# Rikorose/DeepFilterNet

Hardware: AMD Instinct MI355X
Metric: 48 kHz audio frames/sec (hop=480), DeepFilterNet3 enhance() (higher is better)
Workload: dtype f32 (storage and accumulation; GRU projections / recurrences, the fused DF-encoder convolutions and the pointwise halves of the ERB separable convolutions as fp16-split MFMAs: x = hi + lo in f16, hi*hi + hi*lo + lo*hi on v_mfma_f32_16x16x32_f16, ~2^-21 relative; see exact_fp32_ms_per_step); 1 GPU; DeepFilterNet3 (recalled shipped shape, conv_ch=64) enhance(pad=True), batch=256 clips x 10 s @48 kHz per GPU, 1002 STFT frames per clip; batch_per_gpu=256, global_batch=256, parallelism=clips sharded over 1 GPU(s); no collective, inputs_resident_in_hbm=True

## Files before the change

deepfilternet_amd/csrc/dfx_model.hip:

```cpp
#include "dfx_manifest.h"
#include "dfx_nn_kernels.h"

#include <cmath>
#include <functional>
#include <atomic>
#include <map>
#include <mutex>
#include <type_traits>
#include <fcntl.h>
#include <sys/file.h>
#include <sys/stat.h>
#include <unistd.h>

static int check_cfg(const dfx_model_cfg *c) {
    if (!c) DFX_FAIL(DFX_ERR_INVALID_ARG, "null model cfg");
    if (c->conv_ch != 16 && c->conv_ch != 32 && c->conv_ch != 64)
        DFX_FAIL(DFX_ERR_UNSUPPORTED, "conv_ch=%d: the HIP kernels are instantiated for 16, 32, 64", c->conv_ch);
    if (c->emb_hidden_dim != 256 || c->df_hidden_dim != 256) DFX_FAIL(DFX_ERR_UNSUPPORTED, "GRU hidden size must be 256");
    if (c->nb_erb <= 0 || c->nb_erb % 8 || c->nb_erb > 64) DFX_FAIL(DFX_ERR_UNSUPPORTED, "nb_erb must be a multiple of 8, <= 64");
    static_assert(2 * DFX_DEC10_SMEM(64, 64) <= 160 * 1024, "conv_ch <= 64, nb_erb <= 64: dfx_k_erb_dec10 must fit every accepted shape");
    if (c->nb_df <= 0 || c->nb_df % 2 || c->nb_df > c->fft_size / 2 + 1) DFX_FAIL(DFX_ERR_UNSUPPORTED, "nb_df must be even and <= F");
    if (c->df_order <= 0 || c->df_order > 16 || c->df_lookahead < 0 || c->df_lookahead >= c->df_order)
        DFX_FAIL(DFX_ERR_UNSUPPORTED, "need 0 <= df_lookahead < df_order <= 16");
    if (c->conv_lookahead < 0) DFX_FAIL(DFX_ERR_INVALID_ARG, "conv_lookahead < 0");
// ... 296 lines not shown
        if ((f & G.mask[e]) != G.want[e]) continue;
        const float *sp = G.src[e] + b * G.row[e];
        float *dp = G.dst[e] + b * G.row[e];
        for (int64_t i = threadIdx.x; i < G.row[e]; i += blockDim.x) dp[i] = sp[i];
    }
}

__global__ void dfx_k_gate_c0_shift(const unsigned char *flags, float *c0_win, int64_t B, int64_t T, int kt, int64_t frame) {
    const int64_t b = blockIdx.x;
    if (b >= B || !(flags[b] & DFX_GATE_DF)) return;
    float *w = c0_win + (b * T + T - kt) * frame;
    for (int64_t i = (int64_t)blockIdx.y * blockDim.x + threadIdx.x; i < frame; i += (int64_t)gridDim.y * blockDim.x)
        for (int j = 0; j + 1 < kt; ++j) w[j * frame + i] = w[(j + 1) * frame + i];
}

__global__ void dfx_k_gate_hold(const unsigned char *flags, float *win, int64_t cap, int64_t row, int64_t pos, int64_t h, int64_t B) {
    const int64_t b = blockIdx.x;
    if (b >= B || !(flags[b] & DFX_GATE_FROZEN)) return;
    float *w = win + (b * cap + pos) * row;
    for (int64_t i = (int64_t)blockIdx.y * blockDim.x + threadIdx.x; i < row; i += (int64_t)gridDim.y * blockDim.x)
        for (int64_t j = h - 1; j >= 0; --j) w[(j + 1) * row + i] = w[j * row + i];
}

__global__ void dfx_k_gate_pend_commit(const unsigned char *flags, unsigned char *par, int *cnt, int64_t B) {
    const int64_t b = (int64_t)blockIdx.x * blockDim.x + threadIdx.x;
    if (b >= B || !(flags[b] & DFX_GATE_DF)) return;
    par[b] ^= 1;
    cnt[b] += 1;
}

__global__ void dfx_k_gate_finish(const unsigned char *flags, int *skip_counter, float *y, int64_t y_stride, int hop, float *lsnr_out,
                                  int64_t lsnr_stride, int64_t B, int warm) {
    const int64_t b = blockIdx.x;
    if (b >= B) return;
    const unsigned char f = flags[b];
    if (f & DFX_GATE_FROZEN) {
        for (int i = threadIdx.x; i < hop; i += blockDim.x) y[b * y_stride + i] = 0.f;
        if (threadIdx.x == 0 && lsnr_out) lsnr_out[b * lsnr_stride] = (f & DFX_GATE_PAUSED) ? __int_as_float(0x7fc00000) : -15.f;
    } else if (threadIdx.x == 0 && !warm) {
        skip_counter[b] = (f & (DFX_GATE_GAINS | DFX_GATE_ZEROS)) ? 0 : skip_counter[b] + 1;
    }
}

enum { EV_START = 0, EV_C0, EV_C1, EV_C0P, EV_EMB, EV_COEFS, EV_FRONT, EV_DONE, EV_XA, EV_MASK, EV_FIN, EV_TICKET };

struct DfxCan {
    bool fuse_c0 = false;
    bool c0_batch_unfused = false;
    bool c0_h3 = false;
    bool c0_presplit = false;
    bool pw_h3 = false;
    bool fan = false, fan_skp = false;
    bool enc_fan = false;
    bool dfenc = false;
    bool fuse_enc = false;
    bool erb_tail = false;
    bool erb_enc4 = false;
    int df_out = DFX_PLAN_DF_OUT_GGEMM;
};

struct DfxSyncLayout {
    static constexpr size_t LG = (size_t)DFX_MAX_GRU_LAYERS * DFX_SEQ_GMAX;
    static constexpr size_t ready = 0;
    static constexpr size_t emb = 8;
    static constexpr size_t probe = 13;
    static constexpr size_t poison = 14;
    static constexpr size_t done = 16;
    static constexpr size_t pcnt = done + LG;
    static constexpr size_t yprog = pcnt + 16;
    static constexpr size_t giprog = yprog + LG;
    static constexpr size_t xtab = giprog + LG;
    static constexpr size_t xstat = xtab + 3 * LG;
    static constexpr size_t total = xstat + 64;
};

struct dfx_model {
    dfx_model_cfg cfg{};
    float *d_w = nullptr;
    size_t n_w = 0;
    size_t erb0_w = 0, erb0_b = 0;
    PwW erb1, erb2, erb3, dfc0, dfc1, ct3, ct2, ct1;
    size_t co_w = 0, co_ska = 0, co_skb = 0;
    float co_bias = 0.f;
    size_t tail_w0h3 = 0, tail_woh3 = 0;
    float tail_w0_unscale = 1.f, tail_wo_unscale = 1.f;
    GlinW fc_emb, enc_in, enc_out, dec_in, dec_out, dfg_in, df_skip, df_out, enc_skip, dec_skip;
    std::vector<GruW> enc_gru, dec_gru, df_gru;
    size_t lsnr_w = 0;
    float lsnr_b = 0.f;
    size_t fan_w = 0;
    int fan_chunks = 0;
    size_t efan_w1 = 0, efan_w2 = 0;
    int efan_groups = 0;
    size_t dfenc_fc = 0, dfenc_in = 0;
    float dfenc_fc_unscale = 1.f, dfenc_in_unscale = 1.f;
    size_t dfo_h3 = 0;
    float dfo_unscale = 1.f;
    size_t cp_w1 = 0, cp_w2 = 0, cp_b = 0;
    size_t cp_weff = 0, cp_b16 = 0;
    size_t cin_weff = 0, cin_b = 0;
    size_t c0_h3 = 0, dfc1_h3 = 0, cp_h3 = 0;
    float c0_unscale = 1.f, dfc1_unscale = 1.f, cp_unscale = 1.f;
    int cp_G = 0, cp_NO = 0;
    DfxLane *lanes = nullptr;
    struct DfxLaneSet *laneset = nullptr;
    hipEvent_t ev_fork = nullptr;
    hipEvent_t ev_pass = nullptr;
    hipEvent_t ev_gate = nullptr;
    mutable bool pass_pending = false;
    bool enqueue_ahead = false;
    bool concurrent = false;
    int max_chunks = 1;
    int tchunks = 12;
    int tchunk_min = 32;
    bool run_df = true;
    bool exact_fp32 = false;
    DfxCan can;
    unsigned int *d_sync = nullptr;
    unsigned int *d_psync = nullptr;
    mutable unsigned int seq_pbase = 0;
    mutable int64_t passes_ps = 0;
    mutable int64_t passes_pair = 0;
    mutable int64_t last_plan = 0;
    mutable int64_t passes_seq = 0, passes_ev = 0;
    mutable unsigned int seq_base = 0;
    unsigned long long *d_trace = nullptr;
    mutable int trace_dims[3] = {0, 0, 0};
    bool gru_seq = true;
    struct {
        int chunks = 0;
        bool gru_pair_far = false;
        bool gru_pair = true;
        int convp_late = -1;
        int p0_ahead = 3;
        int tail_every = 1;
        int dftail_every = 0;
        bool tail_split = true;
        int64_t convp_elems = (int64_t)1 << 29;
        bool c0_presplit = true;
        bool seq_trace = false;
        char hwq_probe_mode = 0;
        bool erb_enc_split = false;
        int ws_fill = -1;
    } sw;
    unsigned int *d_err = nullptr;
    unsigned int *h_err = nullptr;
    bool check_every_pass = false;
    int spin_limit = DFX_SYNC_SPIN_LIMIT;
    bool hwq_probe_pending = false;
    int hwq_probe = -1;
    const float *p(size_t off) const { return d_w + off; }
};

namespace {
struct Prep {
    const float *blob;
    const DfxManifest &man;
    std::vector<float> out;
    std::string err;
    bool exact_fp32 = false;
    struct Packed {
        bool pw = false, tail = false, c0 = false, fan = false, fan_skp = false, encfan = false, dfenc = false;
        int dfo_tiles = 0;
    } packed;
    const float *get(const std::string &name, const DfxTensor **tt = nullptr) {
        const DfxTensor *t = man.find(name);
        if (!t) {
            err = "tensor not in manifest: " + name;
            return nullptr;
        }
        if (tt) *tt = t;
        return blob + t->offset;
    }
    size_t alloc(size_t n) {
        size_t off = (out.size() + 3) & ~(size_t)3;
        out.resize(off + n, 0.f);
        return off;
    }
    bool bn(const std::string &p, int n, std::vector<float> &scale, std::vector<float> &shift) {
        const float *g = get(p + ".weight"), *b = get(p + ".bias"), *m = get(p + ".running_mean"), *v = get(p + ".running_var");
        if (!g || !b || !m || !v) return false;
        scale.resize(n);
        shift.resize(n);
        for (int i = 0; i < n; ++i) {
            const float s = g[i] / sqrtf(v[i] + 1e-5f);
            scale[i] = s;
            shift[i] = b[i] - m[i] * s;
        }
        return true;
    }
};

bool prep_sep(Prep &P, const std::string &name, int C, PwW &w) {
    const float *dw = P.get(name + ".0.weight"), *pw = P.get(name + ".1.weight");
    std::vector<float> sc, sh;
    if (!dw || !pw || !P.bn(name + ".2", C, sc, sh)) return false;
    w.dw = P.alloc(3 * C);
    w.wt = P.alloc((size_t)C * C);
    w.bias = P.alloc(C);
    for (int c = 0; c < C; ++c)
        for (int j = 0; j < 3; ++j) P.out[w.dw + j * C + c] = dw[c * 3 + j];
    for (int n = 0; n < C; ++n)
        for (int k = 0; k < C; ++k) P.out[w.wt + (size_t)k * C + n] = pw[(size_t)n * C + k] * sc[n];
    for (int n = 0; n < C; ++n) P.out[w.bias + n] = sh[n];
    return true;
}
// ... 286 lines not shown
    }
    const DfxLane &ln = m->lanes[0];
    std::vector<hipStream_t> ss;
    if (ln.gs[1]) ss.push_back(ln.gs[1]);
    for (int i = 0; i < DFX_MAX_GRU_LAYERS; ++i)
        if (ln.ps[i]) ss.push_back(ln.ps[i]);
    for (int i = 0; i < 2; ++i)
        if (ln.ts[i]) ss.push_back(ln.ts[i]);
    unsigned int *cnt = m->d_sync + DfxSyncLayout::probe;
    for (hipStream_t st : ss) dfx_launch(dfx_k_probe_meet, dim3(1), dim3(64), 0, st, cnt, 0u, 1, m->d_err + 9);
    bool okp = hipGetLastError() == hipSuccess;
    for (hipStream_t st : ss) okp = hipStreamSynchronize(st) == hipSuccess && okp;
    m->hwq_probe = 0;
    for (int attempt = 0; attempt < 2 && okp && m->hwq_probe == 0; ++attempt) {
        (void)hipMemset(cnt, 0, sizeof(unsigned int));
        m->h_err[8] = 0u;
        for (hipStream_t st : ss) dfx_launch(dfx_k_probe_meet, dim3(1), dim3(64), 0, st, cnt, (unsigned int)ss.size(), 1 << (16 + 3 * attempt), m->d_err + 8);
        okp = hipGetLastError() == hipSuccess;
        for (hipStream_t st : ss) okp = hipStreamSynchronize(st) == hipSuccess && okp;
        m->hwq_probe = okp && ((volatile unsigned int *)m->h_err)[8] == 0u ? 1 : 0;
    }
    m->h_err[8] = 0u, m->h_err[9] = 0u;
    (void)hipMemset(cnt, 0, sizeof(unsigned int));
    if (ls) ls->hwq_probe = m->hwq_probe;
    if (m->hwq_probe == 0) hwq_probe_fallback(m);
}

namespace {
bool prep_erb_conv0(Prep &P, dfx_model *m) {
    const int C = m->cfg.conv_ch;
    const float *w = P.get("enc.erb_conv0.1.weight");
    std::vector<float> sc, sh;
    if (!w || !P.bn("enc.erb_conv0.2", C, sc, sh)) return false;
    m->erb0_w = P.alloc(9 * C);
    m->erb0_b = P.alloc(C);
    for (int ch = 0; ch < C; ++ch) {
        for (int k = 0; k < 9; ++k) P.out[m->erb0_w + k * C + ch] = w[ch * 9 + k] * sc[ch];
        P.out[m->erb0_b + ch] = sh[ch];
    }
    return true;
}
bool prep_df_conv0(Prep &P, dfx_model *m) {
    const int C = m->cfg.conv_ch;
    const float *w = P.get("enc.df_conv0.1.weight"), *pw = P.get("enc.df_conv0.2.weight");
    std::vector<float> sc, sh;
    if (!w || !pw || !P.bn("enc.df_conv0.3", C, sc, sh)) return false;
    m->cin_weff = P.alloc((size_t)20 * C);
    m->cin_b = P.alloc(C);
    for (int n = 0; n < C; ++n) {
        for (int tap = 0; tap < 9; ++tap)
            for (int ch = 0; ch < 2; ++ch) {
                double acc = 0.0;
                for (int c = ch * (C / 2); c < (ch + 1) * (C / 2); ++c) acc += (double)pw[(size_t)n * C + c] * (double)w[c * 9 + tap];
                P.out[m->cin_weff + (size_t)(tap * 2 + ch) * C + n] = (float)(acc * (double)sc[n]);
            }
        P.out[m->cin_b + n] = sh[n];
    }
    return true;
}
bool prep_lsnr(Prep &P, dfx_model *m) {
    const float *w = P.get("enc.lsnr_fc.0.weight"), *b = P.get("enc.lsnr_fc.0.bias");
    if (!w || !b) return false;
    const int emb = m->cfg.conv_ch * m->cfg.nb_erb / 4;
    m->lsnr_w = P.alloc(emb);
    memcpy(&P.out[m->lsnr_w], w, sizeof(float) * emb);
    m->lsnr_b = b[0];
    return true;
}
bool prep_conv0_out(Prep &P, dfx_model *m) {
    const int C = m->cfg.conv_ch;
    const float *w = P.get("erb_dec.conv0_out.0.weight");
    std::vector<float> sc, sh;
    if (!w || !P.bn("erb_dec.conv0_out.1", 1, sc, sh)) return false;
    m->co_w = P.alloc(3 * C);
    for (int ch = 0; ch < C; ++ch)
        for (int j = 0; j < 3; ++j) P.out[m->co_w + j * C + ch] = w[ch * 3 + j] * sc[0];
    m->co_bias = sh[0];
    return true;
}
void pack_tail_h3(Prep &P, dfx_model *m) {
    const int C = m->cfg.conv_ch;
    if (C % 32 != 0) return;
    const int KC = C / 32;
    const size_t w0 = m->erb0_w, b0 = m->erb0_b, wo = m->co_w;
    m->tail_w0h3 = pack_h3(P, C / 16, [&](int nt, int l, int i) {
        const int k = 8 * (l >> 4) + i, ch = 16 * nt + (l & 15);
        return k < 9 ? P.out[w0 + (size_t)k * C + ch] : (k == 9 ? P.out[b0 + ch] : 0.f);
    }, &m->tail_w0_unscale);
    m->tail_woh3 = pack_h3(P, KC, [&](int kc, int l, int i) {
        const int j = l & 15, e = 8 * kc + i, ch = 16 * (e >> 2) + 4 * (l >> 4) + (e & 3);
        return j < 3 ? P.out[wo + (size_t)j * C + ch] : 0.f;
    }, &m->tail_wo_unscale);
    P.packed.tail = true;
}
bool prep_df_convp(Prep &P, dfx_model *m) {
    const dfx_model_cfg &c = m->cfg;
    const int C = c.conv_ch, kt = c.df_pathway_kernel_size_t, NO = 2 * c.df_order, G = dfx_gcd(C, NO), CG = C / G, OG = NO / G;
    const int idx = kt > 1 ? 1 : 0;
    const bool has_pw = kt > 1;
    const float *w = P.get("df_dec.df_convp." + std::to_string(idx) + ".weight");
    const float *pw = has_pw ? P.get("df_dec.df_convp." + std::to_string(idx + 1) + ".weight") : nullptr;
    std::vector<float> sc, sh;
    if (!w || (has_pw && !pw) || !P.bn("df_dec.df_convp." + std::to_string(idx + (has_pw ? 2 : 1)), NO, sc, sh)) return false;
    m->cp_G = G;
    m->cp_NO = NO;
    m->cp_w1 = P.alloc((size_t)G * kt * CG * 16);
    m->cp_w2 = P.alloc((size_t)NO * NO);
    m->cp_b = P.alloc(NO);
    for (int g = 0; g < G; ++g)
        for (int k = 0; k < kt; ++k)
            for (int ci = 0; ci < CG; ++ci)
                for (int o = 0; o < OG; ++o) {
                    float v = w[(((size_t)(g * OG + o) * CG + ci) * kt + k)];
                    if (!has_pw) v *= sc[g * OG + o];
                    P.out[m->cp_w1 + ((((size_t)g * kt + k) * CG + ci) * 16 + o)] = v;
                }
    for (int n = 0; n < NO; ++n) {
        for (int o = 0; o < NO; ++o) P.out[m->cp_w2 + (size_t)n * NO + o] = has_pw ? pw[(size_t)n * NO + o] * sc[n] : (n == o ? 1.f : 0.f);
        P.out[m->cp_b + n] = sh[n];
    }
    const bool folded = NO <= 16;
    m->cp_weff = P.alloc(folded ? (size_t)kt * C * 16 : 0);
    m->cp_b16 = P.alloc(16);
    for (int k = 0; folded && k < kt; ++k)
        for (int ch = 0; ch < C; ++ch) {
            const int g = ch / CG, ci = ch - g * CG;
            for (int n = 0; n < NO; ++n) {
                double acc = 0.0;
                for (int o = g * OG; o < (g + 1) * OG; ++o) {
                    const double p2 = has_pw ? (double)pw[(size_t)n * NO + o] : (n == o ? 1.0 : 0.0);
                    acc += p2 * (double)w[((size_t)o * CG + ci) * kt + k];
                }
                P.out[m->cp_weff + ((size_t)k * C + ch) * 16 + n] = (float)(acc * (double)sc[n]);
            }
        }
    for (int n = 0; folded && n < NO; ++n) P.out[m->cp_b16 + n] = sh[n];
    return true;
}
void pack_c0_h3(Prep &P, dfx_model *m) {
    const dfx_model_cfg &c = m->cfg;
    const int C = c.conv_ch, kt = c.df_pathway_kernel_size_t;
    if (C % 32 != 0 || 2 * c.df_order > 16) return;
    const int KC = C / 32;
    auto chan = [](int kc, int l, int i) { const int e = 8 * kc + i; return 16 * (e >> 2) + 4 * (l >> 4) + (e & 3); };
    const size_t cin = m->cin_weff, wt1 = m->dfc1.wt, cpw = m->cp_weff;
    m->c0_h3 = pack_h3(P, C / 16, [&](int nt, int l, int i) {
        const int k = 8 * (l >> 4) + i;
        return k < 18 ? P.out[cin + (size_t)k * C + 16 * nt + (l & 15)] : 0.f;
    }, &m->c0_unscale);
    m->dfc1_h3 = pack_h3(P, (C / 16) * KC, [&](int fr, int l, int i) {
        const int nt = fr / KC, kc = fr % KC;
        return P.out[wt1 + (size_t)chan(kc, l, i) * C + 16 * nt + (l & 15)];
    }, &m->dfc1_unscale);
    m->cp_h3 = pack_h3(P, kt * KC, [&](int fr, int l, int i) {
        const int k = fr / KC, kc = fr % KC;
        return P.out[cpw + ((size_t)k * C + chan(kc, l, i)) * 16 + (l & 15)];
    }, &m->cp_unscale);
    P.packed.c0 = true;
}
void pack_dfo_h3(Prep &P, dfx_model *m) {
    const GlinW a = m->df_out;
    const int NO = 2 * m->cfg.df_order, Fd = m->cfg.nb_df;
    if (!(a.Kg <= 32 && a.Kg % 8 == 0 && a.Ng % 2 == 0 && NO % 2 == 0 && Fd % 2 == 0 && (int64_t)a.G * a.Ng == (int64_t)NO * Fd &&
          DFX_DFO_SMEM(NO, Fd) <= (size_t)64 * 1024))
        return;
    const int NU = (a.Ng + 15) / 16;
    m->dfo_h3 = pack_h3(P, a.G * NU, [&](int fr, int l, int i) {
        const int g = fr / NU, u = fr % NU, o = 16 * u + (l & 15), k = 8 * (l >> 4) + i;
        return o < a.Ng && k < a.Kg ? P.out[a.w + ((size_t)g * a.Kg + k) * a.Ng + o] : 0.f;
    }, &m->dfo_unscale);
    P.packed.dfo_tiles = NU;
// ... 165 lines not shown
        } else if (m->sw.hwq_probe_mode != '0') {
            m->hwq_probe_pending = true;
        }
    }
    *out = m;
    return DFX_OK;
}

static void pass_gate_forget(const dfx_model *m);
extern "C" void dfx_model_free(dfx_model *m) {
    if (!m) return;
    pass_gate_forget(m);
    if (m->ev_fork) (void)hipEventDestroy(m->ev_fork);
    if (m->ev_pass) (void)hipEventDestroy(m->ev_pass);
    if (m->ev_gate) (void)hipEventDestroy(m->ev_gate);
    dfx_env_err_words_free(m->h_err);
    if (m->d_sync && m->d_trace) {
        unsigned int n = 0;
        if (hipMemcpy(&n, m->d_sync + DfxSyncLayout::xstat, sizeof(n), hipMemcpyDeviceToHost) == hipSuccess) fprintf(stderr, "[dfx] same-XCD (light) block hand-overs over the model's life: %u\n", n);
    }
    if (m->d_sync) (void)hipFree(m->d_sync);
    if (m->d_psync) (void)hipFree(m->d_psync);
    if (m->d_trace) (void)hipFree(m->d_trace);
    if (m->d_w) (void)hipFree(m->d_w);
    delete m;
}
extern "C" int dfx_model_set_streams(dfx_model *m, int enable) {
    if (!m) DFX_FAIL(DFX_ERR_INVALID_ARG, "null");
    m->concurrent = enable != 0;
    return DFX_OK;
}
extern "C" int dfx_model_set_run_df(dfx_model *m, int enable) {
    if (!m) DFX_FAIL(DFX_ERR_INVALID_ARG, "null");
    m->run_df = enable != 0;
    return DFX_OK;
}
extern "C" int dfx_model_set_pipeline(dfx_model *m, int time_chunks, int min_chunk_frames, int batch_chunks) {
    if (!m || time_chunks < 1 || min_chunk_frames < 1 || batch_chunks < 1) DFX_FAIL(DFX_ERR_INVALID_ARG, "dfx_model_set_pipeline: bad arguments");
    m->tchunks = time_chunks < DFX_MAX_TCHUNKS ? time_chunks : DFX_MAX_TCHUNKS;
    m->tchunk_min = min_chunk_frames;
    m->max_chunks = batch_chunks < DFX_MAX_LANES ? batch_chunks : DFX_MAX_LANES;
    for (int l = 1; l < m->max_chunks; ++l)
        if (!dfx_create_lane(m, l)) DFX_FAIL(DFX_ERR_HIP, "dfx_model_set_pipeline: could not create the streams of lane %d", l);
    return DFX_OK;
}
static int model_poll(const dfx_model *m) {
    unsigned int *h = m->h_err;
    if (!h) return DFX_OK;
    if (!(((volatile unsigned int *)h)[1] | ((volatile unsigned int *)h)[2])) return DFX_OK;
    const unsigned int e1 = __atomic_exchange_n(&h[1], 0u, __ATOMIC_ACQ_REL), e2 = __atomic_exchange_n(&h[2], 0u, __ATOMIC_ACQ_REL);
    if (!(e1 | e2)) return DFX_OK;
    if (e2)
        DFX_FAIL(DFX_ERR_HIP, "dfx: a flag wait of the persistent GRU phase timed out (bounded spin: the streams of the pass did not make progress "
                              "independently — hardware queues shared with other work, or the GPU shared with another process); the results of "
                              "the previous pass on this model are invalid.  DFX_GRU_SEQ=0 selects the event-synchronised form");
    DFX_FAIL(DFX_ERR_UNSUPPORTED, "dfx: an activation of magnitude >= 6e4 reached an fp16-split matrix kernel (GRU / DF-encoder / separable-conv "
                                  "path); the results of the previous pass on this model are invalid.  DFX_EXACT_FP32=1 selects the exact fp32 kernels");
}
extern "C" int dfx_model_poll(const dfx_model *m) {
    if (!m) DFX_FAIL(DFX_ERR_INVALID_ARG, "null");
    return model_poll(m);
}
extern "C" int dfx_model_check(const dfx_model *m) {
    if (!m) DFX_FAIL(DFX_ERR_INVALID_ARG, "null");
    DFX_HIP(hipDeviceSynchronize());
    return model_poll(m);
}
extern "C" int dfx_model_query(const dfx_model *m, int what, int64_t *value) {
    if (!m || !value) DFX_FAIL(DFX_ERR_INVALID_ARG, "dfx_model_query: null");
    switch (what) {
        case DFX_Q_GRU_PERSISTENT:
        case DFX_Q_HWQ_PROBE: {
            std::lock_guard<std::mutex> lk(dfx_enqueue_mu());
            hwq_probe_run(const_cast<dfx_model *>(m));
            *value = what == DFX_Q_HWQ_PROBE ? m->hwq_probe : (m->gru_seq && m->concurrent ? 1 : 0);
            return DFX_OK;
        }
        case DFX_Q_EXACT_FP32: *value = m->exact_fp32 ? 1 : 0; return DFX_OK;
        case DFX_Q_PASSES_PERSISTENT: *value = m->passes_seq; return DFX_OK;
        case DFX_Q_PASSES_TICKET_BUSY: *value = m->passes_ev; return DFX_OK;
        case DFX_Q_SPIN_LIMIT: *value = m->spin_limit; return DFX_OK;
        case DFX_Q_PASSES_C0_PRESPLIT: *value = m->passes_ps; return DFX_OK;
        case DFX_Q_LAST_PLAN: *value = m->last_plan; return DFX_OK;
        case DFX_Q_PASSES_PAIR: *value = m->passes_pair; return DFX_OK;
    }
    DFX_FAIL(DFX_ERR_INVALID_ARG, "dfx_model_query: unknown item %d", what);
}
extern "C" int dfx_model_seq_trace(const dfx_model *m, unsigned long long *out_host, int64_t cap, int *dims) {
    if (!m || !m->d_trace || !out_host || !dims) DFX_FAIL(DFX_ERR_INVALID_ARG, "dfx_model_seq_trace: tracing is off (DFX_SEQ_TRACE=1 at model creation)");
    const int64_t n = (int64_t)m->trace_dims[0] * m->trace_dims[1] * m->trace_dims[2] * 3;
    if (n > cap) DFX_FAIL(DFX_ERR_INVALID_ARG, "dfx_model_seq_trace: buffer too small");
    DFX_HIP(hipMemcpy(out_host, m->d_trace, (size_t)n * 8, hipMemcpyDeviceToHost));
    for (int i = 0; i < 3; ++i) dims[i] = m->trace_dims[i];
    return DFX_OK;
}
extern "C" int dfx_model_cfg_get(const dfx_model *m, dfx_model_cfg *out) {
    if (!m || !out) DFX_FAIL(DFX_ERR_INVALID_ARG, "null");
    *out = m->cfg;
    return DFX_OK;
}

static inline bool dfx_dfenc_ok(const dfx_model *m, int64_t B, int64_t T, int64_t feat_T) {
    const dfx_model_cfg &c = m->cfg;
    const int64_t emb = (int64_t)c.conv_ch * c.nb_erb / 4;
    return m->can.dfenc && B * T * emb < ((int64_t)1 << 31) && B * (feat_T > 0 ? feat_T : T) * c.nb_df < ((int64_t)1 << 29);
}
static inline bool dfx_feat_spec_unread(const dfx_model *m, int64_t B, int64_t T) { return m->can.c0_presplit && dfx_dfenc_ok(m, B, T, 0); }
static inline float *dfx_ws_base(void *workspace) { return reinterpret_cast<float *>(((uintptr_t)workspace + 255) & ~(uintptr_t)255); }

namespace {
struct Ws {
    size_t e0, e1, e2, e3, c0, c1, emb_in, emb, xa, xb, gi, xa2, xb2, gi2, demb, d3, d2, mask, c0p, xdf, coefs, lsnr, skp_e, skp_d, fps, total;
    size_t pgi[DFX_MAX_GRU_LAYERS], py[DFX_MAX_GRU_LAYERS], ph[DFX_MAX_GRU_LAYERS];
};
Ws plan_ws(const dfx_model *m, int64_t R, int64_t B) {
    const dfx_model_cfg &c = m->cfg;
    const bool c0_stored = !m->can.fuse_c0 || m->can.c0_batch_unfused, presplit = m->can.c0_presplit;
    Ws w{};
    size_t off = 0;
    auto take = [&](size_t n) {
        size_t o = off;
        off += (n + 63) & ~(size_t)63;
        return o;
    };
    const size_t C = c.conv_ch, E = c.nb_erb, Fd = c.nb_df, emb = C * E / 4, NO = 2 * c.df_order;
    w.e0 = take(R * E * C);
    w.e1 = take(R * (E / 2) * C);
    w.e2 = take(R * (E / 4) * C);
    w.e3 = take(R * (E / 4) * C);
    w.c0 = c0_stored ? take(R * Fd * C) : 0;
    w.c1 = take(R * (Fd / 2) * C);
    w.emb_in = take(R * emb * (c.enc_concat ? 2 : 1));
    w.emb = take(R * emb);
    w.xa = take(R * 256);
    w.xb = take(R * 256);
    w.gi = take(R * 768);
    w.xa2 = take(R * 256);
    w.xb2 = take(R * 256);
    w.gi2 = take(R * 768);
    w.demb = take(R * emb);
    w.d3 = take(R * (E / 4) * C);
    w.d2 = take(R * (E / 2) * C);
    w.mask = take(R * E);
    w.c0p = take(R * Fd * NO);
    w.xdf = take(R * 256);
    w.coefs = take(R * Fd * NO);
    w.lsnr = take(R);
    w.skp_e = take(c.emb_gru_skip_enc == DFX_SKIP_GROUPEDLINEAR ? R * emb : 0);
    w.skp_d = take(c.emb_gru_skip == DFX_SKIP_GROUPEDLINEAR ? R * emb : 0);
    w.fps = take(presplit ? R * Fd * 2 : 0);
    const int nlayers = 1 + (c.emb_num_layers - 1) + c.df_num_layers;
    for (int l = 0; l < DFX_MAX_GRU_LAYERS; ++l) {
        const bool used = l < nlayers;
        w.pgi[l] = take(used ? R * 768 : 0);
        w.py[l] = take(used ? R * 256 : 0);
        w.ph[l] = take(used ? (B > 0 ? B : R) * 256 : 0);
    }
    w.total = off;
    return w;
}
}

extern "C" int dfx_model_workspace_bytes(const dfx_model *m, int64_t B, int64_t T, int64_t *bytes) {
    if (!m || !bytes || B < 0 || T < 0) DFX_FAIL(DFX_ERR_INVALID_ARG, "dfx_model_workspace_bytes: bad arguments");
    *bytes = (int64_t)(plan_ws(m, B * T, B).total * sizeof(float)) + 256;
    return DFX_OK;
}

#include "dfx_model_launch.h"
#include "dfx_model_forward.h"
#include "dfx_model_stream.h"
#include "dfx_stream_move.h"
#include "dfx_model_enhance.h"
```

deepfilternet_amd/csrc/dfx_model_forward.h:

```cpp
#pragma once

#ifdef DFX_DEV
static int dfx_dev_skip() {
    static const int v = [] { const char *e = getenv("DFX_DEV_SKIP"); return e ? atoi(e) : 0; }();
    return v;
}
static bool dfx_dev_stage(int n) {
    static const int lo = [] { const char *e = getenv("DFX_DEV_STAGE_LO"); return e ? atoi(e) : 0; }();
    static const int hi = [] { const char *e = getenv("DFX_DEV_STAGE_HI"); return e ? atoi(e) : 99; }();
    return n >= lo && n <= hi;
}
#else
static constexpr int dfx_dev_skip() { return 0; }
static constexpr bool dfx_dev_stage(int) { return true; }
#endif

struct TicketGuard {
    bool armed = false;
    ~TicketGuard() {
        if (armed) dfx_ticket_release_cb(nullptr);
    }
};

template <int C>
struct DfxPass {
    const dfx_model *m;
    const dfx_bands *bands;
    const float *spec, *feat_erb, *feat_spec;
    int64_t B, T;
    float atten_lim;
    float *spec_e, *ws;
    hipStream_t s;
    const DfxLane *ln;
    bool signal_front;
    const DfxFinish *fin;
    const DfxStreamCtx *sc;
    const dfx_model_cfg &c;
    int64_t R, t_begin, Rn, featT, t_zero, sstride;
    DfxRowMap rmw;
    int Lk, E, Fd, O, NO, emb, L, kt;
    const int *tzr;
    Ws w{};
    float *e0, *e1, *e2, *e3, *c0, *c1, *emb_in, *embv, *xa, *xb, *gi, *demb, *d3, *d2, *mask, *c0p, *xdf, *coefs, *lsnr, *xa2, *xb2, *gi2, *skp_e, *skp_d;
    bool run_df, fan, fan_skp, par, c0_fused, fuse_h3, fuse_tail, fuse_enc, no_e0, fuse_enc4, enc_fan, dfenc, pipe, use_seq;
    hipStream_t x1, x2;
    hipStream_t fin_s;
    const float *cp_feat, *e0r;
    const uint2 *fps;
    const DfxGate *gate;
    int nenc, ndec, ndf, nl, groups;
    int K = 0;
    int cb[DFX_GS_MAX_CHUNKS + 1];
    int64_t convp_split;
    TicketGuard ticket_guard;

    int plan(float *mask_out, float *lsnr_out, float *coefs_out) {
        R = B * T;
        if (R >= ((int64_t)1 << 31)) DFX_FAIL(DFX_ERR_UNSUPPORTED, "forward: %lld x %lld frames in one call (32-bit row index)", (long long)B, (long long)T);
        t_begin = sc ? sc->H : 0, Rn = B * (T - t_begin);
        featT = sc ? sc->feat_T : 0;
        rmw = sc ? DfxRowMap{T, T - t_begin, t_begin} : DfxRowMap{0, 0, 0};
        Lk = sc ? 0 : c.conv_lookahead;
        t_zero = sc ? sc->t_zero : 0;
        tzr = sc ? sc->t_zero_rows : nullptr;
        w = plan_ws(m, R, B);
        sstride = fin ? fin->spec_stride : 0;
        fin_s = s;
        E = c.nb_erb, Fd = c.nb_df, O = c.df_order, NO = 2 * O, emb = C * E / 4, L = c.conv_lookahead;
        e0 = ws + w.e0, e1 = ws + w.e1, e2 = ws + w.e2, e3 = ws + w.e3, c0 = ws + w.c0, c1 = ws + w.c1;
        emb_in = ws + w.emb_in, embv = ws + w.emb, xa = ws + w.xa, xb = ws + w.xb, gi = ws + w.gi;
        demb = ws + w.demb, d3 = ws + w.d3, d2 = ws + w.d2;
        mask = mask_out ? mask_out : ws + w.mask;
        c0p = ws + w.c0p, xdf = ws + w.xdf;
        coefs = coefs_out ? coefs_out : ws + w.coefs;
        lsnr = lsnr_out ? lsnr_out : ws + w.lsnr;
        xa2 = ws + w.xa2, xb2 = ws + w.xb2, gi2 = ws + w.gi2;
        skp_e = ws + w.skp_e, skp_d = ws + w.skp_d;
        run_df = m->run_df;
        fan = m->can.fan;
        fan_skp = m->can.fan_skp && run_df;
        par = m->concurrent;
        x1 = par ? ln->aux[0] : s, x2 = par ? ln->aux[1] : s;
        c0_fused = m->can.fuse_c0 && !(m->can.c0_batch_unfused && !sc);
        if (sc && !c0_fused) DFX_FAIL(DFX_ERR_UNSUPPORTED, "streaming needs the fused DF encoder (df_pathway_kernel_size_t <= 5, df_order <= 8)");
        cp_feat = c0_fused ? feat_spec : nullptr;
        fuse_h3 = c0_fused && m->can.c0_h3;
        fps = !sc && m->can.c0_presplit ? reinterpret_cast<const uint2 *>(ws + w.fps) : nullptr;
        fuse_tail = m->can.erb_tail, fuse_enc = m->can.fuse_enc;
        no_e0 = fuse_tail && fuse_enc;
        fuse_enc4 = m->can.erb_enc4 && !sc && !m->sw.erb_enc_split;
        e0r = no_e0 ? nullptr : e0;
        if (sc && !fuse_enc) DFX_FAIL(DFX_ERR_UNSUPPORTED, "streaming needs the fused ERB encoder head (nb_erb even and <= 62, a frame's rows within the LDS)");
        gate = sc ? sc->gate : nullptr;
        if (gate && T - t_begin != 1) DFX_FAIL(DFX_ERR_INVALID_ARG, "gated streaming passes carry exactly one new frame");
        kt = c.df_pathway_kernel_size_t;
        convp_split = T;
        enc_fan = m->can.enc_fan;
        dfenc = fuse_h3 && dfx_dfenc_ok(m, B, T, featT);
        K = m->tchunks;
        if (T / K < m->tchunk_min) K = (int)(T / m->tchunk_min);
        nenc = (int)m->enc_gru.size(), ndec = (int)m->dec_gru.size(), ndf = run_df ? (int)m->df_gru.size() : 0;
        pipe = par && !sc && K > 1 && nenc == 1 && 1 + ndec + ndf <= DFX_MAX_GRU_LAYERS && ln == &m->lanes[0];
        nl = 1 + ndec + ndf;
        groups = (int)dfx_ceil_div(B, DFX_GH_ROWS);
        if (pipe && m->gru_seq && m->hwq_probe_pending && groups <= DFX_SEQ_GMAX && nl * groups + 8 <= dfx_env_num_cus())
            hwq_probe_run(const_cast<dfx_model *>(m));
        const bool want_seq = pipe && m->gru_seq && groups <= DFX_SEQ_GMAX && nl * groups + 8 <= dfx_env_num_cus();
        use_seq = want_seq && dfx_ticket_try();
        m->passes_seq += use_seq ? 1 : 0, m->passes_ev += (want_seq && !use_seq) ? 1 : 0;
        ticket_guard.armed = use_seq && dfx_ticket().fd >= 0;
        if (use_seq) {
            const int kbody = m->sw.chunks > 0 ? m->sw.chunks : 12;
            const int64_t body = std::max<int64_t>(dfx_ceil_div(T, (int64_t)kbody), m->tchunk_min);
            K = (int)std::max<int64_t>(1, std::min<int64_t>(dfx_ceil_div(T, body), DFX_GS_MAX_CHUNKS));
        }
        if (pipe)
            for (int i = 0; i <= K; ++i) cb[i] = (int)(T * i / K);
        m->last_plan = (fan ? DFX_PLAN_FAN : 0) | (fan_skp ? DFX_PLAN_FAN_SKP : 0) | (fuse_h3 ? DFX_PLAN_FUSE_H3 : 0) |
                       (c0_fused && fps ? DFX_PLAN_PRESPLIT : 0) | (fuse_tail ? DFX_PLAN_FUSE_TAIL : 0) | (fuse_enc ? DFX_PLAN_FUSE_ENC : 0) |
                       (fuse_enc4 ? DFX_PLAN_FUSE_ENC4 : 0) | (enc_fan ? DFX_PLAN_ENC_FAN : 0) | (dfenc ? DFX_PLAN_DFENC : 0) |
                       (c0_fused ? DFX_PLAN_C0_FUSED : 0) | (pipe ? DFX_PLAN_PIPE : 0) | (use_seq ? DFX_PLAN_USE_SEQ : 0) |
                       DFX_PLAN_FUSE_DEC;
        return DFX_OK;
    }
    void note_df_out(int form) const { m->last_plan = (m->last_plan & ~(int64_t)DFX_PLAN_DF_OUT_MASK) | ((int64_t)form << DFX_PLAN_DF_OUT_SHIFT); }
    int64_t tb(int k) const { return cb[k]; }
    DfxRowMap rmk(int k0, int k) const { return DfxRowMap{T, tb(k + 1) - tb(k0), tb(k0)}; }
    DfxRowMap rmk(int k) const { return rmk(k, k); }
    int64_t Mk(int k0, int k) const { return B * (tb(k + 1) - tb(k0)); }
    int64_t Mk(int k) const { return Mk(k, k); }

    int signal(int e, hipStream_t from) {
        if (par) DFX_HIP(hipEventRecord(ln->ev[e], from));
        return DFX_OK;
    }
    int wait(int e, hipStream_t on) {
        if (par) DFX_HIP(hipStreamWaitEvent(on, ln->ev[e], 0));
        return DFX_OK;
    }
    int ewait(hipEvent_t e, hipStream_t on) {
        DFX_HIP(hipStreamWaitEvent(on, e, 0));
        return DFX_OK;
    }
    int esig(hipEvent_t e, hipStream_t from) {
        DFX_HIP(hipEventRecord(e, from));
        return DFX_OK;
    }
    int enc_skip_res(const float **res, int64_t M, hipStream_t st, DfxRowMap rm) {
        *res = c.emb_gru_skip_enc == DFX_SKIP_IDENTITY ? emb_in : c.emb_gru_skip_enc == DFX_SKIP_GROUPEDLINEAR ? skp_e : nullptr;
        return *res == skp_e ? launch_glin(m, m->enc_skip, emb_in, DFX_ACT_NONE, nullptr, skp_e, M, st, rm) : DFX_OK;
    }
    int enc_out_skip(const float *y, int64_t M, hipStream_t st, DfxRowMap rm) {
        const float *res;
        if (int r = enc_skip_res(&res, M, st, rm)) return r;
        return launch_glin(m, m->enc_out, y, DFX_ACT_RELU, res, embv, M, st, rm);
    }
    int dec_out_skip(const float *y, int64_t M, hipStream_t st, DfxRowMap rm) {
        const float *res = nullptr;
        if (c.emb_gru_skip == DFX_SKIP_IDENTITY) res = embv;
        else if (c.emb_gru_skip == DFX_SKIP_GROUPEDLINEAR) {
            if (int r = launch_glin(m, m->dec_skip, embv, DFX_ACT_NONE, nullptr, skp_d, M, st, rm)) return r;
            res = skp_d;
        }
        return launch_glin(m, m->dec_out, y, DFX_ACT_RELU, res, demb, M, st, rm);
    }
    int emb_fan(const float *y, float *dec_x, int64_t M, hipStream_t st, DfxRowMap rm, const DfxPublish *pub = nullptr) {
        const float *res;
        if (int r = enc_skip_res(&res, M, st, rm)) return r;
        const bool need_emb = c.emb_gru_skip != DFX_SKIP_NONE || (run_df && c.df_gru_skip == DFX_SKIP_IDENTITY);
        return launch_emb_fan(m, y, res, need_emb ? embv : nullptr, dec_x, run_df ? xa2 : nullptr, fan_skp ? xdf : nullptr, lsnr, M, st, rm, embv, pub);
    }
    int df_out_rows(const float *cfeat, const float *cfeat2, int64_t M, hipStream_t st, DfxRowMap rm) {
        if (m->can.df_out != DFX_PLAN_DF_OUT_GGEMM && M > 0 && R * (int64_t)NO * Fd < ((int64_t)1 << 31)) {
            DfxDfOutArgs A;
            A.a = cfeat, A.a2 = cfeat2;
            A.wf = reinterpret_cast<const dfx_h8 *>(m->p(m->dfo_h3));
            A.c0p = c0p, A.out = coefs;
            A.R = M, A.T = T;
            A.G = m->df_out.G, A.Kg = m->df_out.Kg, A.Ng = m->df_out.Ng, A.NO = NO, A.Fd = Fd;
            A.unscale = m->dfo_unscale;
            A.rm = rm;
            A.err = m->d_err;
            const size_t smem = DFX_DFO_SMEM(NO, Fd);
            DfxKScope ks(DFX_K_GGEMM, st);
            const bool resident = m->can.df_out == DFX_PLAN_DF_OUT_RESIDENT;
            note_df_out(m->can.df_out);
            if (resident) {
                DFX_HIP(dfx_env_set_max_dyn_smem((const void *)dfx_k_df_out_h3r<4>, smem));
                dfx_launch(dfx_k_df_out_h3r<4>, dim3((unsigned)nn_grid(dfx_ceil_div(M, 16), 2)), dim3(DFX_DFO_THREADS), smem, st, A);
            } else {
                DFX_HIP(dfx_env_set_max_dyn_smem((const void *)dfx_k_df_out_h3, smem));
                dfx_launch(dfx_k_df_out_h3, dim3((unsigned)nn_grid(dfx_ceil_div(M, 16), 2)), dim3(DFX_DFO_THREADS), smem, st, A);
            }
            DFX_LAUNCH_CHECK();
            return DFX_OK;
        }
        note_df_out(DFX_PLAN_DF_OUT_GGEMM);
        return launch_ggemm(cfeat, m->df_out.G * m->df_out.Kg, m->p(m->df_out.w), m->df_out.G, m->df_out.Kg, m->df_out.Ng, nullptr, DFX_ACT_TANH,
                            c0p, coefs, m->df_out.G * m->df_out.Ng, M, st, NO, Fd, T, rm, cfeat2);
    }
    int erb_dec_convs(int64_t M, DfxRowMap rm, hipStream_t st) {
        int r;
        if (fuse_tail) return launch_erb_tail<C>(m, demb, e3, e2, e1, e0r, mask, M, E, st, rm, feat_erb, T, featT, Lk);
        if ((r = launch_pw<C>(DFX_PW_MODE_DW3, m, m->ct3, demb, e3, d3, M, E / 4, E / 4, 1, st, rm))) return r;
        if ((r = launch_pw<C>(DFX_PW_MODE_DWT3, m, m->ct2, d3, e2, d2, M, E / 4, E / 2, 2, st, rm))) return r;
        return launch_erb_dec10<C>(m, d2, e1, e0, mask, M, E, st, rm);
    }
    int df_skip_identity(const float *y, hipStream_t st) {
        DfxKScope ks(DFX_K_ADD, st);
        dfx_launch(dfx_k_add, dim3((unsigned)nn_grid(dfx_ceil_div(R * 256, 256), 16)), dim3(256), 0, st, y, (const float *)embv, xdf, R * 256);
        DFX_LAUNCH_CHECK();
        return DFX_OK;
    }
    int df_tail_rows(const float *y, int64_t M, DfxRowMap rm, hipStream_t st, bool join_c0p = false) {
        int r;
        const float *cfeat = y, *cfeat2 = nullptr;
        if (fan_skp) {
            cfeat2 = xdf;
        } else if (c.df_gru_skip == DFX_SKIP_GROUPEDLINEAR) {
            if ((r = launch_glin(m, m->df_skip, embv, DFX_ACT_NONE, y, xdf, M, st, rm))) return r;
            cfeat = xdf;
        } else if (c.df_gru_skip == DFX_SKIP_IDENTITY) {
            if ((r = df_skip_identity(y, st))) return r;
            cfeat = xdf;
        }
        if (join_c0p && (r = wait(EV_C0P, st))) return r;
        return df_out_rows(cfeat, cfeat2, M, st, rm);
    }
    int df_tail_identity(const float *y, hipStream_t st) {
        if (int r = df_skip_identity(y, st)) return r;
        note_df_out(DFX_PLAN_DF_OUT_GGEMM);
        return launch_ggemm(xdf, m->df_out.G * m->df_out.Kg, m->p(m->df_out.w), m->df_out.G, m->df_out.Kg, m->df_out.Ng, nullptr, DFX_ACT_TANH,
                            c0p, coefs, m->df_out.G * m->df_out.Ng, R, st, NO, Fd, T);
    }
    int lsnr_all(hipStream_t st) {
        DfxKScope ks(DFX_K_LSNR, st);
        dfx_launch(dfx_k_lsnr, dim3((unsigned)dfx_ceil_div(R * 64, 256)), dim3(256), 0, st, (const float *)embv, m->p(m->lsnr_w), m->lsnr_b,
                   (float)(c.lsnr_max - c.lsnr_min), (float)c.lsnr_min, lsnr, R, emb);
        DFX_LAUNCH_CHECK();
        return DFX_OK;
    }
    int proj_chunk(const GruW &g, int l, int k, const float *xin, hipStream_t st, const DfxPublish *pub = nullptr) {
        if (m->exact_fp32) {
            const int r = launch_proj(xin, m->p(g.wih_t), m->p(g.bias_i), ws + w.pgi[l], Mk(k), 768, st, rmk(k));
            return r || !pub ? r : launch_flag_set(pub->flag, pub->value, st);
        }
        return launch_proj_h3(m, g, xin, ws + w.pgi[l], Mk(k), 768, st, rmk(k), pub);
    }
    int conv_in_df(float *out, int lookahead, int64_t t0, int64_t rows, hipStream_t st) {
        DfxCinArgs A;
        A.feat = feat_spec, A.weff = m->p(m->cin_weff), A.bias = m->p(m->cin_b), A.out = out;
        A.B = B, A.T = T, A.Fin = Fd, A.L = lookahead;
        A.t_begin = t0, A.out_T = T, A.out_toff = t0;
        DfxKScope ks(DFX_K_CONV_IN_DF, st);
        dfx_launch(dfx_k_conv_in_df<C>, dim3((unsigned)nn_grid(dfx_ceil_div(rows * Fd, 64), 8)), dim3(DFX_PW_THREADS), 0, st, A);
        DFX_LAUNCH_CHECK();
        return DFX_OK;
    }
    int df1_range(int64_t t0, int64_t t1, hipStream_t st) {
        if (fuse_h3) return launch_conv01_h3<C>(m, m->dfc1, feat_spec, c1, B, T, Fd, Fd / 2, 2, st, t0, Lk, t1, featT);
        return launch_conv01<C>(m, m->dfc1, feat_spec, c1, B, T, Fd, Fd / 2, 2, st, t0, Lk, t1);
    }
    int convp_range(int64_t t0, int64_t t1, hipStream_t st) {
        if (dfx_dev_skip() & 8) return DFX_OK;
        if (gate && kt > 1 && gate->pend2 && fuse_h3 && t1 - t0 == 1 && t1 == T)
            return dfx_with_kt<2>(kt, [&](auto k) {
                return launch_convp_step<C, decltype(k)::value>(m, feat_spec, c0p, B, T, Fd, NO, st, t_zero, Lk, gate->pend2, 0, false, featT, gate->par, gate->cnt, tzr);
            });
        if (gate && kt > 1) {
            if (kt > 5) DFX_FAIL(DFX_ERR_UNSUPPORTED, "gated streaming needs df_pathway_kernel_size_t <= 5");
            if (int r = conv_in_df(gate->c0_win, Lk, T - 1, B, st)) return r;
            return dfx_with_kt<2>(kt, [&](auto k) { return launch_convp2<C, decltype(k)::value>(m, gate->c0_win, nullptr, c0p, B, T, Fd, NO, st, T - 1, 0, Lk); });
        } else if (fuse_h3 && sc && sc->c0ring && !gate && t1 - t0 == 1 && t1 == T && kt >= 2) {
            sc->c0ring_used = true;
            return dfx_with_kt<2>(kt, [&](auto k) {
                return launch_convp_step<C, decltype(k)::value>(m, feat_spec, c0p, B, T, Fd, NO, st, t_zero, Lk, sc->c0ring, sc->c0slot, sc->c0rebuild, featT, nullptr, nullptr, tzr);
            });
        } else if (fuse_h3) {
            return dfx_with_kt<1>(kt, [&](auto k) { return launch_convp_h3<C, decltype(k)::value>(m, feat_spec, c0p, B, T, Fd, NO, st, t0, t_zero, Lk, t1, featT, tzr, fps); });
        } else if (kt <= 5 && NO <= 16) {
            return dfx_with_kt<1>(kt, [&](auto k) { return launch_convp2<C, decltype(k)::value>(m, c0, cp_feat, c0p, B, T, Fd, NO, st, t0, t_zero, Lk, t1, tzr); });
        }
        DfxCpArgs A;
        A.c0 = c0;
        A.w1 = m->p(m->cp_w1);
        A.w2 = m->p(m->cp_w2);
        A.bias = m->p(m->cp_b);
        A.out = c0p;
        A.B = B;
        A.T = T;
        A.Fd = Fd;
        A.kt = kt;
        A.G = m->cp_G;
        A.NO = NO;
        A.tchunks = (int)dfx_ceil_div(T, DFX_CP_TT);
        A.fchunks = (Fd + DFX_CP_FB - 1) / DFX_CP_FB;
        const int CG = C / A.G;
        const size_t smem = ((size_t)(DFX_CP_TT + A.kt - 1) * DFX_CP_FB * (C + 2) + (size_t)A.G * A.kt * CG * 16 +
                             (size_t)DFX_CP_TT * DFX_CP_FB * NO) * sizeof(float);
        if (smem > 64 * 1024) DFX_HIP(dfx_env_set_max_dyn_smem((const void *)dfx_k_df_convp<C>, smem));
        const int64_t nblk = B * A.tchunks * A.fchunks;
        if (nblk > 0x7fffffff) DFX_FAIL(DFX_ERR_UNSUPPORTED, "df_convp grid too large");
        DfxKScope ks(DFX_K_DF_CONVP, st);
        dfx_launch(dfx_k_df_convp<C>, dim3((unsigned)nblk), dim3(DFX_CP_THREADS), smem, st, A);
        DFX_LAUNCH_CHECK();
        return DFX_OK;
    }
    int erb_range(int64_t t0, int64_t t1, int64_t Rk, DfxRowMap rm, hipStream_t st) {
        int r;
        if (fuse_enc4) return launch_erb_enc4<C>(m, feat_erb, no_e0 ? nullptr : e0, e1, e2, e3, B, T, st, t0, Lk, t1, featT);
        if (fuse_enc) {
            if ((r = launch_erb_enc<C>(m, feat_erb, no_e0 ? nullptr : e0, e1, B, T, st, t0, Lk, t1, featT))) return r;
        } else {
            {
                const int64_t total = R * E * (C / 4);
                DfxKScope ks(DFX_K_CONV_IN_ERB, st);
                dfx_launch(dfx_k_conv_in_erb, dim3((unsigned)nn_grid(dfx_ceil_div(total, 256), 16)), dim3(256), 0, st, feat_erb,
                           m->p(m->erb0_w), m->p(m->erb0_b), e0, B, T, E, C, L);
                DFX_LAUNCH_CHECK();
            }
            if ((r = launch_pw<C>(DFX_PW_MODE_DW3, m, m->erb1, e0, nullptr, e1, R, E, E / 2, 2, st))) return r;
        }
        if ((r = launch_pw<C>(DFX_PW_MODE_DW3, m, m->erb2, e1, nullptr, e2, Rk, E / 2, E / 4, 2, st, rm))) return r;
        return launch_pw<C>(DFX_PW_MODE_DW3, m, m->erb3, e2, nullptr, e3, Rk, E / 4, E / 4, 1, st, rm);
    }
    int emb_range(int64_t Rk, DfxRowMap rm, hipStream_t st) {
        int r;
        if (enc_fan) return launch_enc_fan(m, c1, e3, c.emb_gru_skip_enc != DFX_SKIP_NONE ? emb_in : nullptr, xa, Rk, st, rm);
        if (c.enc_concat) {
            if ((r = stream_copy_rows(e3, emb, emb, 0, emb_in, 2 * emb, emb, R, st))) return r;
            if ((r = launch_ggemm(c1, m->fc_emb.G * m->fc_emb.Kg, m->p(m->fc_emb.w), m->fc_emb.G, m->fc_emb.Kg, m->fc_emb.Ng, nullptr, DFX_ACT_RELU,
                                  nullptr, emb_in + emb, 2 * emb, Rk, st, 0, 0, 1, rm)))
                return r;
        } else if ((r = launch_glin(m, m->fc_emb, c1, DFX_ACT_RELU, e3, emb_in, Rk, st, rm))) return r;
        return launch_glin(m, m->enc_in, emb_in, DFX_ACT_RELU, nullptr, xa, Rk, st, rm);
    }

    int front() {
        int rc;
        if ((rc = signal(EV_START, s)) || (rc = wait(EV_START, x1))) return rc;
        const bool post_behind_convp = sc && sc->df_post && m->run_df;
        if (sc && sc->erb_pre && (rc = sc->erb_pre(s))) return rc;
        if (sc && sc->df_pre && (rc = sc->df_pre(x1))) return rc;
        if (sc && sc->df_post && !post_behind_convp && (rc = sc->df_post(x1))) return rc;
        if (c0_fused) {
            m->passes_ps += fps ? 1 : 0;
            if (fps && !(fin && fin->feat_ps_made) && (rc = dfx_launch_pack_h3(feat_spec, ws + w.fps, R * Fd, m->d_err, x1))) return rc;
            if ((rc = signal(EV_C0, x1)) || (rc = wait(EV_C0, x2))) return rc;
            if (!dfenc && dfx_dev_stage(3) && (rc = df1_range(t_begin, T, x1))) return rc;
        } else {
            if ((rc = conv_in_df(c0, L, 0, R, x1))) return rc;
            if ((rc = signal(EV_C0, x1)) || (rc = wait(EV_C0, x2))) return rc;
            if ((rc = launch_pw<C>(DFX_PW_MODE_DW3, m, m->dfc1, c0, nullptr, c1, R, Fd, Fd / 2, 2, x1))) return rc;
        }
        if ((rc = signal(EV_C1, x1))) return rc;
        if (run_df) {
            const int late_env = m->sw.convp_late;
            const int late_pct = late_env >= 0 ? late_env : (m->exact_fp32 ? 0 : 100);
            convp_split = use_seq && late_pct > 0 ? T - (T - t_begin) * late_pct / 100 : T;
            if (convp_split > t_begin && dfx_dev_stage(1) && (rc = convp_range(t_begin, convp_split, x2))) return rc;
            if (post_behind_convp && (rc = sc->df_post(x2))) return rc;
            if (convp_split >= T && (rc = signal(EV_C0P, x2))) return rc;
        }
        if (dfx_dev_stage(2) && (rc = erb_range(t_begin, T, Rn, rmw, s))) return rc;
        if ((rc = wait(EV_C1, s))) return rc;
        if (dfenc) {
            if (dfx_dev_stage(3) && (rc = launch_df_enc<C>(m, feat_spec, e3, c.emb_gru_skip_enc != DFX_SKIP_NONE ? emb_in : nullptr, xa, B, T, Fd, s, t_begin, Lk, T, featT, fps))) return rc;
        } else if (dfx_dev_stage(3) && (rc = emb_range(Rn, rmw, s))) return rc;
        if (signal_front && (rc = signal(EV_FRONT, s))) return rc;
        return DFX_OK;
    }

    int gru_serial() {
        int rc;
        float *hs_enc = sc ? sc->h_state : nullptr, *hs_dec = sc ? sc->h_state + (int64_t)nenc * B * 256 : nullptr;
        float *hs_df = sc ? sc->h_state + (int64_t)(nenc + ndec) * B * 256 : nullptr;
        float *hn_enc = sc && sc->h_next ? sc->h_next : nullptr, *hn_dec = hn_enc ? hn_enc + (int64_t)nenc * B * 256 : nullptr;
        float *hn_df = hn_enc ? hn_enc + (int64_t)(nenc + ndec) * B * 256 : nullptr;
        const float *y = xa;
        if (dfx_dev_stage(4) && (rc = run_gru_stack(m, m->enc_gru, xa, xa, xb, gi, B, T, &y, s, hs_enc, t_begin, rmw, hn_enc))) return rc;
        float *dec_x = y == xa ? xb : xa;
        if (fan) {
            if (dfx_dev_stage(5) && (rc = emb_fan(y, dec_x, Rn, s, rmw))) return rc;
            if ((rc = signal(EV_EMB, s)) || (rc = wait(EV_EMB, x1))) return rc;
        } else {
            if ((rc = enc_out_skip(y, Rn, s, rmw))) return rc;
            if ((rc = signal(EV_EMB, s)) || (rc = wait(EV_EMB, x1))) return rc;
            if ((rc = lsnr_all(s))) return rc;
        }
        if (gate) {
            dfx_launch(dfx_k_gate_post, dim3((unsigned)dfx_ceil_div(B, 256)), dim3(256), 0, s, (const float *)lsnr, T, gate->thr[0],
                       gate->thr[1], run_df ? gate->thr[2] : -INFINITY, gate->flags, B, gate->channels, gate->thr_rows);
            DFX_LAUNCH_CHECK();
        }
        if (run_df && dfx_dev_stage(6)) {
// ... 508 lines not shown
```

deepfilternet_amd/csrc/dfx_model_launch.h:

```cpp
#pragma once

template <class F>
static int dfx_with_bool(bool b, F &&f) {
    return b ? f(std::true_type{}) : f(std::false_type{});
}
template <int KMIN, class F>
static int dfx_with_kt(int kt, F &&f) {
    if constexpr (KMIN <= 1) {
        if (kt == 1) return f(std::integral_constant<int, 1>{});
    }
    switch (kt) {
        case 2: return f(std::integral_constant<int, 2>{});
        case 3: return f(std::integral_constant<int, 3>{});
        case 4: return f(std::integral_constant<int, 4>{});
        default: return f(std::integral_constant<int, 5>{});
    }
}

static int nn_grid(int64_t tiles, int per_cu) {
    const int64_t cap = (int64_t)dfx_env_num_cus() * per_cu;
    return (int)(tiles < cap ? (tiles > 0 ? tiles : 1) : cap);
}

template <int C>
// ... 196 lines not shown
        DFX_FAIL(DFX_ERR_UNSUPPORTED, "fp16-split df_conv1 needs conv_ch %% 32 == 0");
    } else {
        if (t_end < 0) t_end = T;
        if (B * T >= ((int64_t)1 << 31) || T * Fin >= ((int64_t)1 << 30)) DFX_FAIL(DFX_ERR_UNSUPPORTED, "df_conv0->1: batch too large for one launch (32-bit frame index)");
        DfxC01hArgs A;
        A.t_end = t_end;
        A.feat = feat_spec;
        A.feat_T = feat_T;
        A.w0f = reinterpret_cast<const dfx_h8 *>(m->p(m->c0_h3));
        A.bias0 = m->p(m->cin_b);
        A.dw = m->p(w.dw);
        A.wpf = reinterpret_cast<const dfx_h8 *>(m->p(m->dfc1_h3));
        A.bias = m->p(w.bias);
        A.out = out;
        A.B = B;
        A.T = T;
        A.Fin = Fin;
        A.Fout = Fout;
        A.stride = stride;
        A.L = L < 0 ? m->cfg.conv_lookahead : L;
        A.t_begin = t_begin;
        A.unscale0 = m->c0_unscale;
        A.unscale = m->dfc1_unscale;
        A.err = m->d_err;
        const int grid = nn_grid(dfx_ceil_div(B * (t_end - t_begin) * Fout, 64), 3);
        DfxKScope ks(DFX_K_PWCONV, s);
        dfx_launch(dfx_k_df_conv01_h3<C>, dim3(grid), dim3(DFX_PW_THREADS), 0, s, A);
        DFX_LAUNCH_CHECK();
        return DFX_OK;
    }
}

template <int C>
static int launch_erb_dec10(const dfx_model *m, const float *d2, const float *e1, const float *e0, float *mask, int64_t R, int E,
                            hipStream_t s, DfxRowMap rm) {
    DfxDec10Args A;
    A.x = d2;
    A.skip1 = e1;
    A.sk1_a = m->p(m->ct1.sk_a);
    A.sk1_b = m->p(m->ct1.sk_b);
    A.dw = m->p(m->ct1.dw);
    A.wt = m->p(m->ct1.wt);
    A.bias = m->p(m->ct1.bias);
    A.skip0 = e0;
    A.sk0_a = m->p(m->co_ska);
    A.sk0_b = m->p(m->co_skb);
    A.wo = m->p(m->co_w);
    A.bias_o = m->co_bias;
    A.out = mask;
    A.R = R;
    A.E = E;
    A.rm = rm;
    DfxKScope ks(DFX_K_ERB_DEC, s);
    if (dfx_dec10f_ok(C, E)) {
        DfxDec10fArgs AA;
        AA.a = A;
        const size_t smemf = DFX_DEC10F_SMEM(C, E);
        bool h3 = false;
        if constexpr (C % 32 == 0) {
            if (m->can.pw_h3) {
                h3 = true;
                AA.wt_h3 = reinterpret_cast<const dfx_h8 *>(m->p(m->ct1.wt_h3));
                AA.unscale = m->ct1.unscale;
                AA.err = m->d_err;
            }
        }
        return dfx_with_bool(h3, [&](auto split) {
            auto kern = dfx_k_erb_dec10_f<C, decltype(split)::value && C % 32 == 0>;
            DFX_HIP(dfx_env_set_max_dyn_smem((const void *)kern, smemf));
            dfx_launch(kern, dim3((unsigned)nn_grid(dfx_ceil_div(R, 4), 2)), dim3(256), smemf, s, AA);
            DFX_LAUNCH_CHECK();
            return DFX_OK;
        });
    }
    const size_t smem = DFX_DEC10_SMEM(C, E);
    DFX_HIP(dfx_env_set_max_dyn_smem((const void *)dfx_k_erb_dec10<C>, smem));
    dfx_launch(dfx_k_erb_dec10<C>, dim3((unsigned)nn_grid(dfx_ceil_div(R, 4), 2)), dim3(256), smem, s, A);
    DFX_LAUNCH_CHECK();
    return DFX_OK;
}

template <int C>
static int launch_erb_tail(const dfx_model *m, const float *demb, const float *e3, const float *e2, const float *e1, const float *e0,
                           float *mask, int64_t R, int E, hipStream_t s, DfxRowMap rm, const float *feat_erb = nullptr, int64_t T = 0,
                           int64_t feat_T = 0, int L = 0) {
    if constexpr (C % 32 != 0) {
        DFX_FAIL(DFX_ERR_UNSUPPORTED, "erb tail: conv_ch");
    } else {
        DfxTailArgs A;
        A.demb = demb, A.e3 = e3, A.e2 = e2, A.e1 = e1, A.e0 = e0;
        const PwW *L3[3] = {&m->ct3, &m->ct2, &m->ct1};
        for (int l = 0; l < 3; ++l) {
            A.dw[l] = m->p(L3[l]->dw);
            A.bias[l] = m->p(L3[l]->bias);
            A.wh3[l] = reinterpret_cast<const dfx_h8 *>(m->p(L3[l]->wt_h3));
            A.unscale[l] = L3[l]->unscale;
            A.ska[l] = m->p(L3[l]->sk_a);
            A.skb[l] = m->p(L3[l]->sk_b);
        }
        A.ska[3] = m->p(m->co_ska);
        A.skb[3] = m->p(m->co_skb);
        A.wo = m->p(m->co_w);
        A.woh3 = reinterpret_cast<const dfx_h8 *>(m->p(m->tail_woh3)), A.unscale_wo = m->tail_wo_unscale;
        A.w0h3 = reinterpret_cast<const dfx_h8 *>(m->p(m->tail_w0h3)), A.unscale_w0 = m->tail_w0_unscale;
        A.bias_o = m->co_bias;
        A.out = mask;
        A.R = R;
        A.E = E;
        A.rm = rm;
        A.err = m->d_err;
        if (!e0) {
            if (!feat_erb || T <= 0) DFX_FAIL(DFX_ERR_INVALID_ARG, "erb tail: e0 or the features it is recomputed from");
            A.feat = feat_erb, A.w0 = m->p(m->erb0_w), A.b0 = m->p(m->erb0_b), A.T = T, A.feat_T = feat_T, A.L = L;
        }
        const size_t smem = DFX_TAIL_SMEM(C);
        DFX_HIP(dfx_env_set_max_dyn_smem(e0 ? (const void *)dfx_k_erb_tail<C, false> : (const void *)dfx_k_erb_tail<C, true>, smem));
        DfxKScope ks(DFX_K_ERB_TAIL, s);
        const dim3 grid((unsigned)nn_grid(dfx_ceil_div(R, DFX_TAIL_WAVES), 1));
        if (e0) dfx_launch((dfx_k_erb_tail<C, false>), grid, dim3(64 * DFX_TAIL_WAVES), smem, s, A);
        else dfx_launch((dfx_k_erb_tail<C, true>), grid, dim3(64 * DFX_TAIL_WAVES), smem, s, A);
        DFX_LAUNCH_CHECK();
        return DFX_OK;
    }
}

template <int C>
static int launch_erb_enc(const dfx_model *m, const float *feat_erb, float *e0, float *e1, int64_t B, int64_t T, hipStream_t s,
                          int64_t t_begin = 0, int L = -1, int64_t t_end = -1, int64_t feat_T = 0) {
    const dfx_model_cfg &c = m->cfg;
    if (t_end < 0) t_end = T;
    DfxEncArgs A;
    A.t_end = t_end;
    A.feat = feat_erb;
    A.feat_T = feat_T;
    A.w0 = m->p(m->erb0_w);
    A.b0 = m->p(m->erb0_b);
    A.dw = m->p(m->erb1.dw);
    A.wt = m->p(m->erb1.wt);
    A.bias = m->p(m->erb1.bias);
    A.e0 = e0;
    A.e1 = e1;
    A.B = B;
    A.T = T;
    A.E = c.nb_erb;
    A.L = L < 0 ? c.conv_lookahead : L;
    A.t_begin = t_begin;
    const size_t smem = DFX_ENC_SMEM(C, c.nb_erb);
    DfxKScope ks(DFX_K_ERB_ENC, s);
    const dim3 grid((unsigned)nn_grid(dfx_ceil_div(B * (t_end - t_begin), 4), 2));
    if constexpr (C % 32 == 0) {
        if (m->can.pw_h3) {
            A.wt_h3 = reinterpret_cast<const dfx_h8 *>(m->p(m->erb1.wt_h3));
            A.unscale = m->erb1.unscale;
            A.err = m->d_err;
            DFX_HIP(dfx_env_set_max_dyn_smem((const void *)dfx_k_erb_enc<C, true>, smem));
            dfx_launch(dfx_k_erb_enc<C, true>, grid, dim3(256), smem, s, A);
            DFX_LAUNCH_CHECK();
            return DFX_OK;
        }
    }
    DFX_HIP(dfx_env_set_max_dyn_smem((const void *)dfx_k_erb_enc<C, false>, smem));
    dfx_launch(dfx_k_erb_enc<C, false>, grid, dim3(256), smem, s, A);
    DFX_LAUNCH_CHECK();
    return DFX_OK;
}

template <int C>
static int launch_erb_enc4(const dfx_model *m, const float *feat_erb, float *e0, float *e1, float *e2, float *e3, int64_t B, int64_t T,
                           hipStream_t s, int64_t t_begin = 0, int L = -1, int64_t t_end = -1, int64_t feat_T = 0) {
    if constexpr (C % 32 != 0) {
        DFX_FAIL(DFX_ERR_UNSUPPORTED, "erb enc4: conv_ch");
    } else {
        const dfx_model_cfg &c = m->cfg;
        if (t_end < 0) t_end = T;
        const int64_t R = B * (t_end - t_begin);
        if (R <= 0) return DFX_OK;
        DfxEnc4Args A;
        A.feat = feat_erb;
        A.feat_T = feat_T;
        A.w0 = m->p(m->erb0_w);
        A.b0 = m->p(m->erb0_b);
        const PwW *L3[3] = {&m->erb1, &m->erb2, &m->erb3};
        for (int l = 0; l < 3; ++l) {
            A.dw[l] = m->p(L3[l]->dw);
            A.bias[l] = m->p(L3[l]->bias);
            A.wh3[l] = reinterpret_cast<const dfx_h8 *>(m->p(L3[l]->wt_h3));
            A.unscale[l] = L3[l]->unscale;
        }
        A.e0 = e0, A.e1 = e1, A.e2 = e2, A.e3 = e3;
        A.B = B;
        A.T = T;
        A.E = c.nb_erb;
        A.L = L < 0 ? c.conv_lookahead : L;
        A.t_begin = t_begin;
        A.t_end = t_end;
        A.err = m->d_err;
        const size_t smem = DFX_ENC4_SMEM(C, c.nb_erb);
        DFX_HIP(dfx_env_set_max_dyn_smem((const void *)dfx_k_erb_enc4<C>, smem));
        DfxKScope ks(DFX_K_ERB_ENC, s);
        const dim3 grid((unsigned)nn_grid(dfx_ceil_div(R, DFX_ENC4_WAVES), 1));
        dfx_launch(dfx_k_erb_enc4<C>, grid, dim3(64 * DFX_ENC4_WAVES), smem, s, A);
        DFX_LAUNCH_CHECK();
        return DFX_OK;
    }
}

template <int C>
static int launch_conv01(const dfx_model *m, const PwW &w, const float *feat_spec, float *out, int64_t B, int64_t T, int Fin,
                         int Fout, int stride, hipStream_t s, int64_t t_begin = 0, int L = -1, int64_t t_end = -1) {
    if (t_end < 0) t_end = T;
    DfxC01Args A;
    A.t_end = t_end;
    A.feat = feat_spec;
    A.weff0 = m->p(m->cin_weff);
    A.bias0 = m->p(m->cin_b);
    A.dw = m->p(w.dw);
    A.wt = m->p(w.wt);
    A.bias = m->p(w.bias);
    A.out = out;
    A.B = B;
    A.T = T;
    A.Fin = Fin;
    A.Fout = Fout;
    A.stride = stride;
    A.L = L < 0 ? m->cfg.conv_lookahead : L;
    A.t_begin = t_begin;
    const int grid = nn_grid(dfx_ceil_div(B * (t_end - t_begin) * Fout, 64), 8);
    DfxKScope ks(DFX_K_PWCONV, s);
    dfx_launch(dfx_k_df_conv01<C>, dim3(grid), dim3(DFX_PW_THREADS), 0, s, A);
    DFX_LAUNCH_CHECK();
    return DFX_OK;
}

static int launch_ggemm(const float *a, int lda, const float *w, int G, int Kg, int Ng, const float *bias, int act,
                        const float *res, float *out, int ldo, int64_t M, hipStream_t s, int perm_inner = 0, int perm_F = 0,
                        int64_t perm_T = 1, DfxRowMap rm = DfxRowMap{0, 0, 0}, const float *a2 = nullptr) {
    if (M <= 0) return DFX_OK;
    if (Kg % 4 || Ng % 4 || lda % 4) DFX_FAIL(DFX_ERR_UNSUPPORTED, "grouped GEMM needs K, N, lda multiples of 4 (got %d, %d, %d)", Kg, Ng, lda);
    DfxGgArgs A;
    A.a = a;
    A.a2 = a2;
    A.w = w;
    A.bias = bias;
    A.res = res;
    A.out = out;
    A.M = M;
    A.lda = lda;
    A.ldo = ldo;
    A.G = G;
    A.Kg = Kg;
    A.Ng = Ng;
    A.act = act;
    A.perm_inner = perm_inner;
    A.perm_F = perm_F;
    A.perm_T = perm_T;
    A.rm = rm;
    const int BN = Ng <= 16 ? 16 : (Ng <= 32 ? 32 : 64);
    A.ntn = (Ng + BN - 1) / BN;
    const int64_t nblk = dfx_ceil_div(dfx_ceil_div(M, DFX_GG_BM), 8) * 8 * (int64_t)(G * A.ntn);
    if (nblk > 0x7fffffff) DFX_FAIL(DFX_ERR_UNSUPPORTED, "grouped GEMM grid too large");
    const dim3 grid((unsigned)nblk);
    DfxKScope ks(DFX_K_GGEMM, s);
    if (BN == 16) dfx_launch(dfx_k_ggemm<16>, grid, dim3(DFX_GG_THREADS), 0, s, A);
    else if (BN == 32) dfx_launch(dfx_k_ggemm<32>, grid, dim3(DFX_GG_THREADS), 0, s, A);
    else dfx_launch(dfx_k_ggemm<64>, grid, dim3(DFX_GG_THREADS), 0, s, A);
    DFX_LAUNCH_CHECK();
    return DFX_OK;
}
static int launch_proj(const float *a, const float *w, const float *bias, float *out, int64_t M, int N, hipStream_t s,
                       DfxRowMap rm = DfxRowMap{0, 0, 0}) {
    if (M <= 0) return DFX_OK;
    if (N % DFX_PJ_BN) return launch_ggemm(a, 256, w, 1, 256, N, bias, DFX_ACT_NONE, nullptr, out, N, M, s, 0, 0, 1, rm);
    DfxPjArgs A;
    A.rm = rm;
    A.a = a;
    A.w = w;
    A.bias = bias;
    A.out = out;
    A.M = M;
// ... 285 lines not shown
```

deepfilternet_amd/csrc/dfx_nn_kernels.h:

```cpp
#pragma once

#include "dfx_common.h"

#include <type_traits>

#define DFX_ACT_NONE 0
#define DFX_ACT_RELU 1
#define DFX_ACT_TANH 2
#define DFX_ACT_SIGMOID 3

static __device__ __forceinline__ float dfx_sigmoid(float x) { return 1.f / (1.f + expf(-x)); }
static __device__ __forceinline__ float dfx_act(float v, int act) {
    if (act == DFX_ACT_RELU) return fmaxf(v, 0.f);
    if (act == DFX_ACT_TANH) return tanhf(v);
    if (act == DFX_ACT_SIGMOID) return dfx_sigmoid(v);
    return v;
}

static __device__ __forceinline__ float dfx_row256_scale_split(const float4 (&raw)[16], dfx_h8 (&xh)[8], dfx_h8 (&xl)[8]) {
    float mx = 0.f;
#pragma unroll
    for (int i = 0; i < 16; ++i) mx = fmaxf(mx, fmaxf(fmaxf(fabsf(raw[i].x), fabsf(raw[i].y)), fmaxf(fabsf(raw[i].z), fabsf(raw[i].w))));
    mx = fmaxf(mx, __shfl_xor(mx, 16));
    mx = fmaxf(mx, __shfl_xor(mx, 32));
// ... 1518 lines not shown
                      : make_float4(0.f, 0.f, 0.f, 0.f);
    float areg[H3 ? 1 : NT][H3 ? 1 : CPL];
    dfx_h8 ahi[NT][KC], alo[NT][KC];
    float4 biasr[NT];
    float amax = 0.f;
    if constexpr (H3) dfx_chain_load_w_h3<C>(A.wt_h3, A.bias, lane, ahi, alo, biasr);
    else dfx_chain_load_w<C>(A.wt, A.bias, lane, areg, biasr);
    __syncthreads();
    const int64_t nitems = (A.R + G - 1) / G;
    const int nin4 = nrow_in * C4, nout4 = npos * C4, fin4 = A.Fin * C4, fout4 = A.Fout * C4;
    const float4 *x4 = reinterpret_cast<const float4 *>(A.x);
    const float4 *s4 = reinterpret_cast<const float4 *>(A.skip);
    float4 *o4 = reinterpret_cast<float4 *>(A.out);
    float4 xr[NVI], sr[SKIP ? NVI : 1];
    const float inv_fin4 = 1.0f / (float)fin4, inv_fout = 1.0f / (float)A.Fout;
    auto issue = [&](int64_t item) {
        const int64_t base = item * G;
        const DfxRowBase rb = dfx_row_base(A.rm, base);
        int ln = lane;
        DFX_OPAQUE(ln);
        const float4 *xq = x4, *sq = s4;
#pragma unroll
        for (int i = 0; i < NVI; ++i) {
            const int idx = ln + 64 * i;
            xr[i] = make_float4(0.f, 0.f, 0.f, 0.f);
            if (SKIP) sr[i] = make_float4(0.f, 0.f, 0.f, 0.f);
            if (idx < nin4) {
                const int fr = dfx_div_small(idx, fin4, inv_fin4);
                const int64_t rl = base + fr;
                if (rl < A.R) {
                    const int64_t off = dfx_row_at(A.rm, base, rb, fr) * fin4 + (idx - fr * fin4);
                    xr[i] = xq[off];
                    if (SKIP) sr[i] = sq[off];
                }
            }
        }
    };
    int64_t item = (int64_t)blockIdx.x * 4 + wave;
    if (item < nitems) issue(item);
    static_assert(64 % C4 == 0, "channel quad of a lane must not depend on the load index");
    const float4 ska = sks[lane % C4], skb = sks[C4 + lane % C4];
    for (; item < nitems; item += (int64_t)gridDim.x * 4) {
#pragma unroll
        for (int i = 0; i < NVI; ++i) {
            const int idx = lane + 64 * i;
            if (idx < nin4) {
                const int row = idx / C4, c4 = idx - row * C4;
                float4 v = xr[i];
                if (SKIP) {
                    const float4 sv = sr[i], a = ska, bb = skb;
                    v.x += fmaxf(a.x * sv.x + bb.x, 0.f);
                    v.y += fmaxf(a.y * sv.y + bb.y, 0.f);
                    v.z += fmaxf(a.z * sv.z + bb.z, 0.f);
                    v.w += fmaxf(a.w * sv.w + bb.w, 0.f);
                }
                *reinterpret_cast<float4 *>(sin + row * LD + 4 * c4) = v;
            }
        }
        const int64_t next = item + (int64_t)gridDim.x * 4;
        if (next < nitems) issue(next);
        DFX_WAVE_SYNC();
        auto epi = [&](int p, bool valid, int nt, float4 v) {
            if (valid) *reinterpret_cast<float4 *>(sout + p * LD + 16 * nt + 4 * q) = v;
        };
        if constexpr (H3) dfx_chain_stage_h3<C, MODE>(sin, A.Fin, A.Fout, A.stride, npos, dws, ahi, alo, biasr, A.unscale, amax, lane, epi);
        else dfx_chain_stage<C, MODE>(sin, A.Fin, A.Fout, A.stride, npos, dws, areg, biasr, lane, epi);
        DFX_WAVE_SYNC();
        const int64_t obase = item * G;
        const DfxRowBase orb = dfx_row_base(A.rm, obase);
#pragma unroll
        for (int i = 0; i < DFX_PWF_MAXV; ++i) {
            const int idx = lane + 64 * i;
            if (idx < nout4) {
                const int p = idx / C4, c4 = idx - p * C4;
                const int fr = dfx_div_small(p, A.Fout, inv_fout);
                const int64_t rl = obase + fr;
                if (rl < A.R) o4[dfx_row_at(A.rm, obase, orb, fr) * fout4 + (idx - fr * fout4)] = *reinterpret_cast<const float4 *>(sout + p * LD + 4 * c4);
            }
        }
    }
    if (H3 && amax >= DFX_H3_LIMIT && A.err) dfx_raise(A.err + 1);
}

struct DfxEncArgs {
    const float *feat;
    const float *w0, *b0;
    const float *dw, *wt, *bias;
    float *e0, *e1;
    int64_t B, T;
    int E, L;
    int64_t t_begin, t_end;
    const dfx_h8 *wt_h3 = nullptr;
    float unscale = 1.f;
    unsigned int *err = nullptr;
    int64_t feat_T = 0;
};
#define DFX_ENC_FS(E) (3 * ((E) + 2))
#define DFX_ENC_WAVE_FLOATS(C, E) ((E) * ((C) + 4) + DFX_ENC_FS(E) + 2)
#define DFX_ENC_SMEM(C, E) ((size_t)(3 * (C) / 4) * 16 + (size_t)4 * ((DFX_ENC_WAVE_FLOATS(C, E) + 3) / 4 * 4) * 4)

template <int C, bool H3 = false>
__global__ void __launch_bounds__(256, 2) dfx_k_erb_enc(DfxEncArgs A) {
    constexpr int NT = C / 16, CPL = C / 4, LD = C + 4, C4 = C / 4, KC = H3 ? C / 32 : 1;
    DFX_DYN_SMEM(float4, sm4);
    const int tid = threadIdx.x, lane = tid & 63, wave = tid >> 6, q = lane >> 4;
    const int E = A.E, E1 = E / 2, EP = E + 2;
    float4 *dws = sm4;
    float *s0 = reinterpret_cast<float *>(sm4 + 3 * C4) + (size_t)wave * ((DFX_ENC_WAVE_FLOATS(C, E) + 3) / 4 * 4);
    float *fs = s0 + E * LD;
    for (int i = tid; i < 3 * C4; i += 256) dws[i] = reinterpret_cast<const float4 *>(A.dw)[i];
    float a1[H3 ? 1 : NT][H3 ? 1 : CPL];
    dfx_h8 ahi[NT][KC], alo[NT][KC];
    float4 b1[NT];
    float amax = 0.f;
    if constexpr (H3) dfx_chain_load_w_h3<C>(A.wt_h3, A.bias, lane, ahi, alo, b1);
    else dfx_chain_load_w<C>(A.wt, A.bias, lane, a1, b1);
    const int c4 = lane % C4, pslot = lane / C4, pstep = 64 / C4;
    float4 wv[9];
#pragma unroll
    for (int k = 0; k < 9; ++k) wv[k] = reinterpret_cast<const float4 *>(A.w0)[k * C4 + c4];
    const float4 bv = reinterpret_cast<const float4 *>(A.b0)[c4];
    __syncthreads();
    const int64_t Tn = A.t_end - A.t_begin, R = A.B * Tn;
    const int64_t rstep = (int64_t)gridDim.x * 4;
    float fx[3];
    auto fetch = [&](int64_t rl) {
        const int64_t b = rl / Tn, t = A.t_begin + (rl - b * Tn);
#pragma unroll
        for (int k = 0; k < 3; ++k) {
            const int i = lane + 64 * k, kt = i / EP, fp = i - kt * EP;
            const int64_t tau = t - 2 + kt, tin = tau + A.L;
            float v = 0.f;
            if (rl < R && i < 3 * EP && fp >= 1 && fp <= E && tau >= 0 && tin < A.T) v = A.feat[(b * (A.feat_T > 0 ? A.feat_T : A.T) + tin) * E + fp - 1];
            fx[k] = v;
        }
    };
    int64_t rl = (int64_t)blockIdx.x * 4 + wave;
    fetch(rl);
    for (; rl < R; rl += rstep) {
        const int64_t r = (rl / Tn) * A.T + A.t_begin + rl % Tn;
#pragma unroll
        for (int k = 0; k < 3; ++k)
            if (lane + 64 * k < 3 * EP) fs[lane + 64 * k] = fx[k];
        fetch(rl + rstep);
        DFX_WAVE_SYNC();
        for (int p = pslot; p < E; p += pstep) {
            float4 acc = bv;
#pragma unroll
            for (int kt = 0; kt < 3; ++kt)
#pragma unroll
                for (int kf = 0; kf < 3; ++kf) {
                    const float x = fs[kt * EP + p + kf];
                    const float4 ww = wv[kt * 3 + kf];
                    acc.x += ww.x * x;
                    acc.y += ww.y * x;
                    acc.z += ww.z * x;
                    acc.w += ww.w * x;
                }
            const float4 o = make_float4(fmaxf(acc.x, 0.f), fmaxf(acc.y, 0.f), fmaxf(acc.z, 0.f), fmaxf(acc.w, 0.f));
            if (A.e0) reinterpret_cast<float4 *>(A.e0 + (r * E + p) * C)[c4] = o;
            *reinterpret_cast<float4 *>(s0 + p * LD + 4 * c4) = o;
        }
        DFX_WAVE_SYNC();
        auto epi = [&](int p, bool valid, int nt, float4 o) {
            if (valid) *reinterpret_cast<float4 *>(A.e1 + (r * E1 + p) * C + 16 * nt + 4 * q) = o;
        };
        if constexpr (H3) dfx_chain_stage_h3<C, DFX_PW_MODE_DW3>(s0, E, E1, 2, E1, dws, ahi, alo, b1, A.unscale, amax, lane, epi);
        else dfx_chain_stage<C, DFX_PW_MODE_DW3>(s0, E, E1, 2, E1, dws, a1, b1, lane, epi);
        DFX_WAVE_SYNC();
    }
    if (H3 && amax >= DFX_H3_LIMIT && A.err) dfx_raise(A.err + 1);
}

struct DfxDec10Args {
    const float *x;
    const float *skip1;
    const float *sk1_a, *sk1_b;
    const float *dw;
    const float *wt;
    const float *bias;
    const float *skip0;
    const float *sk0_a, *sk0_b;
    const float *wo;
    float bias_o;
    float *out;
    int64_t R;
    int E;
    DfxRowMap rm;
};
#define DFX_DEC10_WAVE_FLOATS(C, E) ((E) * ((C) + 4) + 4 * (E))
#define DFX_DEC10_SMEM(C, E) ((size_t)(3 * (C) / 4 + 4 * (C) / 4 + 3 * (C) / 4) * 16 + (size_t)4 * DFX_DEC10_WAVE_FLOATS(C, E) * 4)

template <int C>
__global__ void __launch_bounds__(256, 2) dfx_k_erb_dec10(DfxDec10Args A) {
    constexpr int NT = C / 16, CPL = C / 4, V4 = CPL / 4, LD = C + 4, C4 = C / 4;
    DFX_DYN_SMEM(float4, sm4);
    const int tid = threadIdx.x, lane = tid & 63, wave = tid >> 6, q = lane >> 4, jl = lane & 15;
    const int E = A.E, E1 = E / 2;
    float4 *dws = sm4;
    float4 *sks = dws + 3 * C4;
    float4 *wos = sks + 4 * C4;
    float *strip = reinterpret_cast<float *>(wos + 3 * C4) + (size_t)wave * DFX_DEC10_WAVE_FLOATS(C, E);
    float *V = strip + E * LD;
    for (int i = tid; i < 3 * C4; i += 256) {
        dws[i] = reinterpret_cast<const float4 *>(A.dw)[i];
        wos[i] = reinterpret_cast<const float4 *>(A.wo)[i];
    }
    for (int i = tid; i < C4; i += 256) {
        sks[i] = reinterpret_cast<const float4 *>(A.sk1_a)[i];
        sks[C4 + i] = reinterpret_cast<const float4 *>(A.sk1_b)[i];
        sks[2 * C4 + i] = reinterpret_cast<const float4 *>(A.sk0_a)[i];
        sks[3 * C4 + i] = reinterpret_cast<const float4 *>(A.sk0_b)[i];
    }
    float areg[NT][CPL];
    float4 biasr[NT];
    dfx_chain_load_w<C>(A.wt, A.bias, lane, areg, biasr);
    __syncthreads();
    for (int64_t rl = (int64_t)blockIdx.x * 4 + wave; rl < A.R; rl += (int64_t)gridDim.x * 4) {
        const int64_t r = dfx_row(A.rm, rl);
        for (int p0 = 0; p0 < E; p0 += 16) {
            const int fo = p0 + jl;
            const bool valid = fo < E;
            float4 s0v[NT];
#pragma unroll
            for (int nt = 0; nt < NT; ++nt)
                s0v[nt] = valid ? *reinterpret_cast<const float4 *>(A.skip0 + (r * E + fo) * C + 16 * nt + 4 * q) : make_float4(0.f, 0.f, 0.f, 0.f);
            float u[CPL];
#pragma unroll
            for (int i = 0; i < CPL; ++i) u[i] = 0.f;
#pragma unroll
            for (int j = 0; j < 3; ++j) {
                const int num = fo + 1 - j, fi = num >> 1;
                if (valid && num >= 0 && (num & 1) == 0 && fi < E1) {
                    const int64_t off = (r * E1 + fi) * C + CPL * q;
                    const float4 *xp = reinterpret_cast<const float4 *>(A.x + off);
                    const float4 *sp = reinterpret_cast<const float4 *>(A.skip1 + off);
#pragma unroll
                    for (int v = 0; v < V4; ++v) {
                        float4 xv = xp[v];
                        const float4 sv = sp[v], a = sks[V4 * q + v], bb = sks[C4 + V4 * q + v];
                        xv.x += fmaxf(a.x * sv.x + bb.x, 0.f);
                        xv.y += fmaxf(a.y * sv.y + bb.y, 0.f);
                        xv.z += fmaxf(a.z * sv.z + bb.z, 0.f);
                        xv.w += fmaxf(a.w * sv.w + bb.w, 0.f);
                        const float4 w = dws[j * C4 + V4 * q + v];
                        u[4 * v + 0] += w.x * xv.x;
// ... 105 lines not shown
        }
#pragma unroll
        for (int i = 0; i < 8; ++i) {
            const int idx = lane + 64 * i;
            s0r[i] = make_float4(0.f, 0.f, 0.f, 0.f);
            if (idx < n0) s0r[i] = s04[r * n0 + idx];
        }
    };
    int64_t rl = (int64_t)blockIdx.x * 4 + wave;
    if (rl < A.R) issue(rl);
    static_assert(64 % C4 == 0, "channel quad of a lane must not depend on the load index");
    for (; rl < A.R; rl += (int64_t)gridDim.x * 4) {
        const int64_t r = dfx_row(A.rm, rl);
        int lq = lane % C4;
        DFX_OPAQUE(lq);
        const float4 sk1a = sks[lq], sk1b = sks[C4 + lq], sk0a = sks[2 * C4 + lq], sk0b = sks[3 * C4 + lq];
#pragma unroll
        for (int i = 0; i < 4; ++i) {
            const int idx = lane + 64 * i;
            if (idx < n1) {
                const int row = idx / C4, c4 = idx - row * C4;
                float4 v = xr[i];
                const float4 sv = s1r[i], a = sk1a, bb = sk1b;
                v.x += fmaxf(a.x * sv.x + bb.x, 0.f);
                v.y += fmaxf(a.y * sv.y + bb.y, 0.f);
                v.z += fmaxf(a.z * sv.z + bb.z, 0.f);
                v.w += fmaxf(a.w * sv.w + bb.w, 0.f);
                *reinterpret_cast<float4 *>(sin + row * LD + 4 * c4) = v;
            }
        }
#pragma unroll
        for (int i = 0; i < 8; ++i) {
            const int idx = lane + 64 * i;
            if (idx < n0) {
                const int row = idx / C4, c4 = idx - row * C4;
                const float4 sv = s0r[i], a = sk0a, bb = sk0b;
                *reinterpret_cast<float4 *>(strip + row * LD + 4 * c4) =
                    make_float4(fmaxf(a.x * sv.x + bb.x, 0.f), fmaxf(a.y * sv.y + bb.y, 0.f), fmaxf(a.z * sv.z + bb.z, 0.f), fmaxf(a.w * sv.w + bb.w, 0.f));
            }
        }
        const int64_t next = rl + (int64_t)gridDim.x * 4;
        if (next < A.R) issue(next);
        DFX_WAVE_SYNC();
        auto epi = [&](int p, bool valid, int nt, float4 d1) {
            if (valid) {
                float4 *dst = reinterpret_cast<float4 *>(strip + p * LD + 16 * nt + 4 * q);
                const float4 e = *dst;
                *dst = make_float4(d1.x + e.x, d1.y + e.y, d1.z + e.z, d1.w + e.w);
            }
        };
        if constexpr (H3) dfx_chain_stage_h3<C, DFX_PW_MODE_DWT3>(sin, E1, E, 2, E, dws, ahi, alo, biasr, AA.unscale, amax, lane, epi);
        else dfx_chain_stage<C, DFX_PW_MODE_DWT3>(sin, E1, E, 2, E, dws, areg, biasr, lane, epi);
        DFX_WAVE_SYNC();
        for (int i = lane; i < 3 * E; i += 64) {
            const int p = i / 3, j = i - 3 * p;
            const float4 *xrow = reinterpret_cast<const float4 *>(strip + p * LD);
            float acc = 0.f;
#pragma unroll 4
            for (int c = 0; c < C4; ++c) {
                const float4 x = xrow[c], w = wos[j * C4 + c];
                acc += w.x * x.x;
                acc += w.y * x.y;
                acc += w.z * x.z;
                acc += w.w * x.w;
            }
            V[i] = acc;
        }
        DFX_WAVE_SYNC();
        for (int f = lane; f < E; f += 64) {
            float acc = A.bias_o + V[f * 3 + 1];
            if (f > 0) acc += V[(f - 1) * 3 + 0];
            if (f < E - 1) acc += V[(f + 1) * 3 + 2];
            A.out[r * E + f] = dfx_sigmoid(acc);
        }
        DFX_WAVE_SYNC();
    }
    if (H3 && amax >= DFX_H3_LIMIT && AA.err) dfx_raise(AA.err + 1);
}

#define DFX_TAIL_WAVES 12
#define DFX_TAIL_WAVE_FLOATS(C) (32 * ((C) + 4))
#define DFX_TAIL_TAB4(C) (3 * 3 * (C) / 4 + 4 * 2 * (C) / 4 + 3 * (C) / 4)
#define DFX_TAIL_WFRAG(C) ((size_t)((C) / 16) * ((C) / 32) * 2 * 64)
#define DFX_TAIL_W0_4(C) (((C) / 16) * 2 * 32 + ((C) / 32) * 2 * 16)
#define DFX_TAIL_SMEM(C) ((size_t)(DFX_TAIL_TAB4(C) + DFX_TAIL_W0_4(C)) * 16 + 3 * DFX_TAIL_WFRAG(C) * 16 + (size_t)DFX_TAIL_WAVES * DFX_TAIL_WAVE_FLOATS(C) * 4)
static __host__ __device__ __forceinline__ bool dfx_tail_ok(int C, int E) {
    return (C == 32 || C == 64) && E == 32 && DFX_TAIL_SMEM(C) <= (size_t)160 * 1024;
}
struct DfxTailArgs {
    const float *demb, *e3, *e2, *e1, *e0;
    const float *dw[3], *bias[3];
    const dfx_h8 *wh3[3];
    float unscale[3];
    const float *ska[4], *skb[4];
    const float *wo;
    const dfx_h8 *woh3;
    const dfx_h8 *w0h3;
    float unscale_wo, unscale_w0;
    float bias_o;
    float *out;
    int64_t R;
    int E;
    DfxRowMap rm;
    unsigned int *err;
    const float *feat = nullptr;
    const float *w0 = nullptr, *b0 = nullptr;
    int64_t T = 0, feat_T = 0;
    int L = 0;
};
template <int C, int MODE, int FB = C / 16, typename Epi>
static __device__ __forceinline__ void dfx_chain_tile_h3_lds(const float *in, int Fin, int stride, int p0, int npos, const float4 *dws,
                                                             const dfx_h8 *wfr, const float4 *bias4, float unscale, float &amax, int lane, Epi &&epi) {
    constexpr int CPL = C / 4, NT = C / 16, KC = C / 32, V4 = CPL / 4, LD = C + 4;
    const int q = lane >> 4, jl = lane & 15;
    const int fo = p0 + jl;
    const bool valid = fo < npos;
    float u[CPL];
#pragma unroll
    for (int i = 0; i < CPL; ++i) u[i] = 0.f;
#pragma unroll
    for (int j = 0; j < 3; ++j) {
        int fi;
        bool ok;
        if (MODE == DFX_PW_MODE_DW3) {
            fi = fo * stride + j - 1;
            ok = fi >= 0 && fi < Fin;
        } else {
            const int num = fo + 1 - j;
            fi = num >> 1;
            ok = num >= 0 && (num & 1) == 0 && fi < Fin;
        }
        if (valid && ok) {
            const float4 *xp = reinterpret_cast<const float4 *>(in + fi * LD + CPL * q);
#pragma unroll
            for (int v = 0; v < V4; ++v) {
                const float4 xv = xp[v];
                const float4 w = dws[j * (C / 4) + V4 * q + v];
                u[4 * v + 0] += w.x * xv.x;
                u[4 * v + 1] += w.y * xv.y;
                u[4 * v + 2] += w.z * xv.z;
                u[4 * v + 3] += w.w * xv.w;
            }
        }
    }
    dfx_h8 bhi[KC], blo[KC];
#pragma unroll
    for (int kc = 0; kc < KC; ++kc) dfx_split8_g(u + 8 * kc, bhi[kc], blo[kc], amax);
    f32x4 acc[NT];
#pragma unroll
    for (int nt = 0; nt < NT; ++nt) acc[nt] = f32x4{0.f, 0.f, 0.f, 0.f};
    static_assert(NT % FB == 0, "whole batches of channel tiles");
#pragma unroll
    for (int kc = 0; kc < KC; ++kc) {
#pragma unroll
        for (int n0 = 0; n0 < NT; n0 += FB) {
            dfx_h8 ahi[FB], alo[FB];
#pragma unroll
            for (int d = 0; d < FB; ++d) {
                ahi[d] = wfr[((size_t)((n0 + d) * KC + kc) * 2 + 0) * 64 + lane];
                alo[d] = wfr[((size_t)((n0 + d) * KC + kc) * 2 + 1) * 64 + lane];
            }
#pragma unroll
            for (int d = 0; d < FB; ++d) {
                acc[n0 + d] = dfx_mfma_16x16x32_f16(alo[d], bhi[kc], acc[n0 + d]);
                acc[n0 + d] = dfx_mfma_16x16x32_f16(ahi[d], blo[kc], acc[n0 + d]);
                acc[n0 + d] = dfx_mfma_16x16x32_f16(ahi[d], bhi[kc], acc[n0 + d]);
            }
        }
    }
#pragma unroll
    for (int nt = 0; nt < NT; ++nt) {
        const float4 bz = bias4[4 * nt + q];
        epi(fo, valid, nt,
            make_float4(fmaxf(acc[nt][0] * unscale + bz.x, 0.f), fmaxf(acc[nt][1] * unscale + bz.y, 0.f), fmaxf(acc[nt][2] * unscale + bz.z, 0.f),
                        fmaxf(acc[nt][3] * unscale + bz.w, 0.f)));
    }
}
template <int C, bool RE0 = false>
__global__ void __launch_bounds__(64 * DFX_TAIL_WAVES, 1) dfx_k_erb_tail(DfxTailArgs A) {
    constexpr int LD = C + 4, C4 = C / 4, NTH = 64 * DFX_TAIL_WAVES;
    constexpr int E = 32, E1 = 16, E4 = 8;
    constexpr int N3 = E4 * C4, N1 = E1 * C4, N0T = 16 * C4;
    constexpr int NV3 = (N3 + 63) / 64, NV1 = (N1 + 63) / 64, NV0 = (N0T + 63) / 64;
    DFX_DYN_SMEM(float4, sm4);
    const int tid = threadIdx.x, lane = tid & 63, wave = tid >> 6, q = lane >> 4;
    constexpr int NT = C / 16, KC = C / 32;
    float4 *dws = sm4;
    float4 *sks = dws + 9 * C4;
    float4 *bis = sks + 8 * C4;
    dfx_h8 *w0f = reinterpret_cast<dfx_h8 *>(bis + 3 * C4);
    dfx_h8 *wof = w0f + NT * 2 * 32;
    dfx_h8 *wfr = w0f + DFX_TAIL_W0_4(C);
    float *X = reinterpret_cast<float *>(wfr + 3 * DFX_TAIL_WFRAG(C)) + (size_t)wave * DFX_TAIL_WAVE_FLOATS(C);
    float *Y = X + 16 * LD;
#pragma unroll
    for (int l = 0; l < 3; ++l) {
        for (int i = tid; i < 3 * C4; i += NTH) dws[l * 3 * C4 + i] = reinterpret_cast<const float4 *>(A.dw[l])[i];
        for (int i = tid; i < C4; i += NTH) bis[l * C4 + i] = reinterpret_cast<const float4 *>(A.bias[l])[i];
        for (int i = tid; i < (int)DFX_TAIL_WFRAG(C); i += NTH) wfr[l * DFX_TAIL_WFRAG(C) + i] = A.wh3[l][i];
    }
#pragma unroll
    for (int pth = 0; pth < 4; ++pth)
        for (int i = tid; i < C4; i += NTH) {
            sks[pth * 2 * C4 + i] = reinterpret_cast<const float4 *>(A.ska[pth])[i];
            sks[pth * 2 * C4 + C4 + i] = reinterpret_cast<const float4 *>(A.skb[pth])[i];
        }
    constexpr bool re0 = RE0;
    if (re0) {
        for (int i = tid; i < NT * 2 * 32; i += NTH) w0f[i] = A.w0h3[(i >> 5) * 64 + (i & 31)];
    }
    for (int i = tid; i < KC * 2 * 16; i += NTH) wof[i] = A.woh3[(i >> 4) * 64 + 16 * ((i & 15) >> 2) + (i & 3)];
    __syncthreads();
    const float4 *pd = reinterpret_cast<const float4 *>(A.demb), *p3 = reinterpret_cast<const float4 *>(A.e3), *p2 = reinterpret_cast<const float4 *>(A.e2),
                 *p1 = reinterpret_cast<const float4 *>(A.e1), *p0 = reinterpret_cast<const float4 *>(A.e0);
    const float4 z4 = make_float4(0.f, 0.f, 0.f, 0.f);
    float4 rd[NV3], r3[NV3], r2[NV3];
    auto issue = [&](int64_t r) {
#pragma unroll
        for (int i = 0; i < NV3; ++i) {
            const int idx = lane + 64 * i;
            rd[i] = r3[i] = r2[i] = z4;
            if (idx < N3) rd[i] = pd[r * N3 + idx], r3[i] = p3[r * N3 + idx], r2[i] = p2[r * N3 + idx];
        }
    };
    auto path = [](float4 sv, float4 a, float4 b) {
        return make_float4(fmaxf(a.x * sv.x + b.x, 0.f), fmaxf(a.y * sv.y + b.y, 0.f), fmaxf(a.z * sv.z + b.z, 0.f), fmaxf(a.w * sv.w + b.w, 0.f));
    };
    auto add_into = [&](float *strip, int prow0) {
        return [=](int p, bool valid, int nt, float4 d) {
            if (valid) {
                float4 *dst = reinterpret_cast<float4 *>(strip + (p - prow0) * LD + 16 * nt + 4 * q);
                const float4 e = *dst;
                *dst = make_float4(d.x + e.x, d.y + e.y, d.z + e.z, d.w + e.w);
            }
        };
    };
    static_assert(64 % C4 == 0, "channel quad of a lane must not depend on the load index");
    float amax = 0.f;
    int64_t rl = (int64_t)blockIdx.x * DFX_TAIL_WAVES + dfx_wave_uniform(wave);
    if (rl < A.R) issue(dfx_row(A.rm, rl));
    for (; rl < A.R; rl += (int64_t)gridDim.x * DFX_TAIL_WAVES) {
        const int64_t r = dfx_row(A.rm, rl);
        int lq = lane % C4;
        DFX_OPAQUE(lq);
        float4 r1[NV1];
        int l1 = lane;
        DFX_OPAQUE(l1);
#pragma unroll
        for (int i = 0; i < NV1; ++i) {
            const int idx = l1 + 64 * i;
            r1[i] = idx < N1 ? p1[r * N1 + idx] : z4;
        }
        float fxr[3] = {0.f, 0.f, 0.f};
        if (re0) {
            const uint32_t cb = (uint32_t)r / (uint32_t)A.T;
            const int64_t ct = r - (int64_t)cb * A.T, fT = A.feat_T > 0 ? A.feat_T : A.T;
#pragma unroll
            for (int kt = 0; kt < 3; ++kt) {
                const int64_t tau = ct - 2 + kt, tin = tau + A.L;
                if (lane >= 1 && lane <= E && tau >= 0 && tin < A.T) fxr[kt] = A.feat[((int64_t)cb * fT + tin) * E + lane - 1];
            }
        }
        {
            const float4 a3 = sks[lq], b3 = sks[C4 + lq], a2 = sks[2 * C4 + lq], b2 = sks[3 * C4 + lq];
#pragma unroll
            for (int i = 0; i < NV3; ++i) {
                const int idx = lane + 64 * i;
                if (idx < N3) {
                    const int row = idx / C4, c4 = idx - row * C4;
                    const float4 pv = path(r3[i], a3, b3);
                    *reinterpret_cast<float4 *>(X + row * LD + 4 * c4) = make_float4(rd[i].x + pv.x, rd[i].y + pv.y, rd[i].z + pv.z, rd[i].w + pv.w);
                    *reinterpret_cast<float4 *>(X + (E4 + row) * LD + 4 * c4) = path(r2[i], a2, b2);
                }
            }
        }
        DFX_WAVE_SYNC();
        dfx_chain_tile_h3_lds<C, DFX_PW_MODE_DW3>(X, E4, 1, 0, E4, dws, wfr, bis, A.unscale[0], amax, lane, add_into(X + E4 * LD, 0));
        {
            const float4 a1 = sks[4 * C4 + lq], b1 = sks[5 * C4 + lq];
#pragma unroll
            for (int i = 0; i < NV1; ++i) {
                const int idx = lane + 64 * i;
                if (idx < N1) {
                    const int row = idx / C4, c4 = idx - row * C4;
                    *reinterpret_cast<float4 *>(Y + row * LD + 4 * c4) = path(r1[i], a1, b1);
                }
            }
        }
        DFX_WAVE_SYNC();
        dfx_chain_tile_h3_lds<C, DFX_PW_MODE_DWT3>(X + E4 * LD, E4, 2, 0, E1, dws + 3 * C4, wfr + DFX_TAIL_WFRAG(C), bis + C4, A.unscale[1], amax, lane,
                                                   add_into(Y, 0));
        DFX_WAVE_SYNC();
        const float4 a0 = sks[6 * C4 + lq], b0 = sks[7 * C4 + lq];
#pragma unroll
        for (int t = 0; t < 2; ++t) {
            if constexpr (re0) {
                int jl = lane & 15;
                DFX_OPAQUE(jl);
                float xk[8];
#pragma unroll
                for (int i = 0; i < 8; ++i) xk[i] = __shfl(fxr[i / 3], 16 * t + jl + i % 3);
                const float x8 = __shfl(fxr[2], 16 * t + jl + 2);
#pragma unroll
                for (int i = 0; i < 8; ++i) xk[i] = q == 0 ? xk[i] : 0.f;
                if (q == 1) xk[0] = x8, xk[1] = 1.f;
                dfx_h8 ph, pl;
                dfx_split8_g(xk, ph, pl, amax);
                int l32 = lane & 31;
                DFX_OPAQUE(l32);
                f32x4 acc0[NT];
#pragma unroll
                for (int nt = 0; nt < NT; ++nt) acc0[nt] = dfx_mfma_16x16x32_f16(w0f[(nt * 2 + 1) * 32 + l32], ph, f32x4{0.f, 0.f, 0.f, 0.f});
#pragma unroll
                for (int nt = 0; nt < NT; ++nt) acc0[nt] = dfx_mfma_16x16x32_f16(w0f[(nt * 2 + 0) * 32 + l32], pl, acc0[nt]);
                DFX_OPAQUE(l32);
#pragma unroll
                for (int nt = 0; nt < NT; ++nt) acc0[nt] = dfx_mfma_16x16x32_f16(w0f[(nt * 2 + 0) * 32 + l32], ph, acc0[nt]);
                DFX_MFMA_GUARD();
#pragma unroll
                for (int nt = 0; nt < NT; ++nt) {
                    const float4 a0q = sks[6 * C4 + 4 * nt + q], b0q = sks[7 * C4 + 4 * nt + q];
                    const float4 ev = make_float4(fmaxf(acc0[nt][0] * A.unscale_w0, 0.f), fmaxf(acc0[nt][1] * A.unscale_w0, 0.f),
                                                  fmaxf(acc0[nt][2] * A.unscale_w0, 0.f), fmaxf(acc0[nt][3] * A.unscale_w0, 0.f));
                    *reinterpret_cast<float4 *>(X + jl * LD + 16 * nt + 4 * q) = path(ev, a0q, b0q);
                }
            } else {
#pragma unroll
                for (int i = 0; i < NV0; ++i) {
                    const int idx = lane + 64 * i;
                    if (idx < N0T) {
                        const int row = idx / C4, c4 = idx - row * C4;
                        *reinterpret_cast<float4 *>(X + row * LD + 4 * c4) = path(p0[(r * 2 + t) * N0T + idx], a0, b0);
                    }
                }
            }
            if (t == 1) {
                const int64_t next = rl + (int64_t)gridDim.x * DFX_TAIL_WAVES;
                if (next < A.R) issue(dfx_row(A.rm, next));
            }
            DFX_WAVE_SYNC();
            float sv[8];
            f32x4 va = f32x4{0.f, 0.f, 0.f, 0.f}, vb = va, vc = va;
            int lw = 4 * q + ((lane & 15) < 3 ? (lane & 15) : 3);
            DFX_OPAQUE(lw);
            dfx_chain_tile_h3_lds<C, DFX_PW_MODE_DWT3, (C >= 64 ? C / 32 : C / 16)>(Y, E1, 2, 16 * t, E, dws + 6 * C4, wfr + 2 * DFX_TAIL_WFRAG(C), bis + 2 * C4, A.unscale[2], amax, lane,
                                                       [&](int p, bool, int nt, float4 d) {
                                                           const float4 e = *reinterpret_cast<const float4 *>(X + (p - 16 * t) * LD + 16 * nt + 4 * q);
                                                           const int o = 4 * (nt & 1);
                                                           sv[o + 0] = d.x + e.x, sv[o + 1] = d.y + e.y, sv[o + 2] = d.z + e.z, sv[o + 3] = d.w + e.w;
                                                           if (nt & 1) {
                                                               const int kc = nt >> 1;
                                                               dfx_h8 sh, sl;
                                                               dfx_split8_g(sv, sh, sl, amax);
                                                               const dfx_h8 woh = wof[(kc * 2 + 0) * 16 + lw], wol = wof[(kc * 2 + 1) * 16 + lw];
                                                               va = dfx_mfma_16x16x32_f16(wol, sh, va);
                                                               vb = dfx_mfma_16x16x32_f16(woh, sl, vb);
                                                               vc = dfx_mfma_16x16x32_f16(woh, sh, vc);
                                                           }
                                                       });
            DFX_MFMA_GUARD();
            const f32x4 vj = (va + vb) + vc;
            DFX_WAVE_SYNC();
            if (lane < 16) {
                float *Vp = t == 0 ? Y : X;
                int lv = lane;
                DFX_OPAQUE(lv);
#pragma unroll
                for (int j = 0; j < 3; ++j) {
                    const int i = lv * 3 + j;
                    Vp[(i >> 2) * LD + C + (i & 3)] = vj[j] * A.unscale_wo;
                }
            }
        }
        DFX_WAVE_SYNC();
        if (lane < E) {
            auto V = [&](int p, int j) -> float {
                const int i = (p & 15) * 3 + j;
                return (p < 16 ? Y : X)[(i >> 2) * LD + C + (i & 3)];
            };
            int f = lane;
            DFX_OPAQUE(f);
            float acc = A.bias_o + V(f, 1);
            if (f > 0) acc += V(f - 1, 0);
            if (f < E - 1) acc += V(f + 1, 2);
            A.out[r * E + f] = dfx_sigmoid(acc);
        }
        DFX_WAVE_SYNC();
    }
    if (amax >= DFX_H3_LIMIT && A.err) dfx_raise(A.err + 1);
}

#define DFX_ENC4_WAVES 12
#define DFX_ENC4_TAB4(C) (3 * 3 * (C) / 4 + 3 * (C) / 4)
#define DFX_ENC4_WAVE_FLOATS(C, E) ((E) * ((C) + 4) + (DFX_ENC_FS(E) + 3) / 4 * 4)
#define DFX_ENC4_SMEM(C, E) ((size_t)DFX_ENC4_TAB4(C) * 16 + 3 * DFX_TAIL_WFRAG(C) * 16 + (size_t)DFX_ENC4_WAVES * DFX_ENC4_WAVE_FLOATS(C, E) * 4)
static __host__ __device__ __forceinline__ bool dfx_enc4_ok(int C, int E) {
    return (C == 32 || C == 64) && E == 32 && DFX_ENC4_SMEM(C, E) <= (size_t)160 * 1024;
}
struct DfxEnc4Args {
    const float *feat;
    const float *w0, *b0;
    const float *dw[3], *bias[3];
    const dfx_h8 *wh3[3];
    float unscale[3];
    float *e0, *e1, *e2, *e3;
    int64_t B, T;
    int E, L;
    int64_t t_begin, t_end;
    int64_t feat_T;
    unsigned int *err;
};
template <int C, int N4>
static __device__ __forceinline__ void dfx_enc4_store_rows(const float *strip, float4 *dst, int lane) {
    constexpr int NV = N4 / 64, C4 = C / 4, LD = C + 4;
    static_assert(N4 % 64 == 0, "whole 16-byte pieces per lane");
    int ln = lane;
    DFX_OPAQUE(ln);
    float4 v[NV];
#pragma unroll
    for (int i = 0; i < NV; ++i) {
        const int idx = ln + 64 * i, row = idx / C4, k4 = idx - row * C4;
        v[i] = *reinterpret_cast<const float4 *>(strip + row * LD + 4 * k4);
    }
#pragma unroll
    for (int i = 0; i < NV; ++i) dst[ln + 64 * i] = v[i];
}
template <int C>
__global__ void __launch_bounds__(64 * DFX_ENC4_WAVES, 1) dfx_k_erb_enc4(DfxEnc4Args A) {
    constexpr int LD = C + 4, C4 = C / 4, NTH = 64 * DFX_ENC4_WAVES;
    DFX_DYN_SMEM(float4, sm4);
    const int tid = threadIdx.x, lane = tid & 63, wave = tid >> 6, q = lane >> 4;
    constexpr int E = 32, E1 = E / 2, E2 = E / 4, EP = E + 2;
    float4 *dws = sm4;
    float4 *bis = dws + 9 * C4;
    dfx_h8 *wfr = reinterpret_cast<dfx_h8 *>(bis + 3 * C4);
    float *S0 = reinterpret_cast<float *>(wfr + 3 * DFX_TAIL_WFRAG(C)) + (size_t)wave * DFX_ENC4_WAVE_FLOATS(C, E);
    float *S1 = S0, *S2 = S0 + E1 * LD, *S3 = S2 + E2 * LD;
    float *fs = S0 + E * LD;
#pragma unroll
    for (int l = 0; l < 3; ++l) {
        for (int i = tid; i < 3 * C4; i += NTH) dws[l * 3 * C4 + i] = reinterpret_cast<const float4 *>(A.dw[l])[i];
        for (int i = tid; i < C4; i += NTH) bis[l * C4 + i] = reinterpret_cast<const float4 *>(A.bias[l])[i];
        for (int i = tid; i < (int)DFX_TAIL_WFRAG(C); i += NTH) wfr[l * DFX_TAIL_WFRAG(C) + i] = A.wh3[l][i];
    }
    static_assert(64 % C4 == 0, "channel quad of a lane must not depend on the load index");
    constexpr int PP = E / (64 / C4);
    const int c4 = lane % C4, pbase = (lane / C4) * PP;
    float4 wv[9];
#pragma unroll
    for (int k = 0; k < 9; ++k) wv[k] = reinterpret_cast<const float4 *>(A.w0)[k * C4 + c4];
    const float4 bv = reinterpret_cast<const float4 *>(A.b0)[c4];
    __syncthreads();
    const uint32_t Tn = (uint32_t)(A.t_end - A.t_begin);
    const int64_t R = A.B * (int64_t)Tn, fT = A.feat_T > 0 ? A.feat_T : A.T;
    const int64_t rstep = (int64_t)gridDim.x * DFX_ENC4_WAVES;
    float fx[3];
    auto fetch = [&](int64_t rl) {
        const uint32_t b = (uint32_t)rl / Tn;
        const int64_t t = A.t_begin + ((uint32_t)rl - b * Tn);
#pragma unroll
        for (int k = 0; k < 3; ++k) {
            const int i = lane + 64 * k, kt = i / EP, fp = i - kt * EP;
            const int64_t tau = t - 2 + kt, tin = tau + A.L;
            float v = 0.f;
            if (rl < R && i < 3 * EP && fp >= 1 && fp <= E && tau >= 0 && tin < A.T) v = A.feat[((int64_t)b * fT + tin) * E + fp - 1];
            fx[k] = v;
        }
    };
    auto into = [&](float *strip) {
        return [=](int p, bool valid, int nt, float4 o) {
            if (valid) *reinterpret_cast<float4 *>(strip + p * LD + 16 * nt + 4 * q) = o;
        };
    };
    float amax = 0.f;
    int64_t rl = (int64_t)blockIdx.x * DFX_ENC4_WAVES + dfx_wave_uniform(wave);
    fetch(rl);
    for (; rl < R; rl += rstep) {
        const uint32_t cb = (uint32_t)rl / Tn;
        const int64_t r = (int64_t)cb * A.T + A.t_begin + ((uint32_t)rl - cb * Tn);
#pragma unroll
        for (int k = 0; k < 3; ++k)
            if (lane + 64 * k < 3 * EP) fs[lane + 64 * k] = fx[k];
        fetch(rl + rstep);
        DFX_WAVE_SYNC();
        static_assert(PP % 4 == 0, "whole groups of four positions per lane");
#pragma unroll 1
        for (int p4 = pbase; p4 < pbase + PP; p4 += 4) {
            float xw[3][6];
#pragma unroll
            for (int kt = 0; kt < 3; ++kt)
#pragma unroll
                for (int i = 0; i < 6; ++i) xw[kt][i] = fs[kt * EP + p4 + i];
#pragma unroll
            for (int it = 0; it < 4; ++it) {
                const int p = p4 + it;
                float4 acc = bv;
#pragma unroll
                for (int kt = 0; kt < 3; ++kt)
#pragma unroll
                    for (int kf = 0; kf < 3; ++kf) {
                        const float x = xw[kt][it + kf];
                        const float4 ww = wv[kt * 3 + kf];
                        acc.x += ww.x * x;
                        acc.y += ww.y * x;
                        acc.z += ww.z * x;
                        acc.w += ww.w * x;
                    }
                const float4 o = make_float4(fmaxf(acc.x, 0.f), fmaxf(acc.y, 0.f), fmaxf(acc.z, 0.f), fmaxf(acc.w, 0.f));
                if (A.e0) reinterpret_cast<float4 *>(A.e0 + (r * E + p) * C)[c4] = o;
                *reinterpret_cast<float4 *>(S0 + p * LD + 4 * c4) = o;
            }
        }
        DFX_WAVE_SYNC();
        dfx_chain_tile_h3_lds<C, DFX_PW_MODE_DW3>(S0, E, 2, 0, E1, dws, wfr, bis, A.unscale[0], amax, lane, [=](int p, bool valid, int nt, float4 o) {
            if (nt == 0) DFX_WAVE_SYNC();
            if (valid) *reinterpret_cast<float4 *>(S1 + p * LD + 16 * nt + 4 * q) = o;
        });
        DFX_WAVE_SYNC();
        dfx_enc4_store_rows<C, E1 * C4>(S1, reinterpret_cast<float4 *>(A.e1) + r * (E1 * C4), lane);
        dfx_chain_tile_h3_lds<C, DFX_PW_MODE_DW3>(S1, E1, 2, 0, E2, dws + 3 * C4, wfr + DFX_TAIL_WFRAG(C), bis + C4, A.unscale[1], amax, lane, into(S2));
        DFX_WAVE_SYNC();
        dfx_enc4_store_rows<C, E2 * C4>(S2, reinterpret_cast<float4 *>(A.e2) + r * (E2 * C4), lane);
        dfx_chain_tile_h3_lds<C, DFX_PW_MODE_DW3>(S2, E2, 1, 0, E2, dws + 6 * C4, wfr + 2 * DFX_TAIL_WFRAG(C), bis + 2 * C4, A.unscale[2], amax, lane, into(S3));
        DFX_WAVE_SYNC();
        dfx_enc4_store_rows<C, E2 * C4>(S3, reinterpret_cast<float4 *>(A.e3) + r * (E2 * C4), lane);
        DFX_WAVE_SYNC();
    }
    if (amax >= DFX_H3_LIMIT && A.err) dfx_raise(A.err + 1);
}

#define DFX_CP_TT 8
#define DFX_CP_FB 16
#define DFX_CP_THREADS 256
struct DfxCpArgs {
    const float *c0;
    const float *w1;
    const float *w2;
    const float *bias;
    float *out;
    int64_t B, T;
    int Fd, kt, G, NO;
    int tchunks, fchunks;
};

template <int C>
__global__ void __launch_bounds__(DFX_CP_THREADS) dfx_k_df_convp(DfxCpArgs A) {
    constexpr int LDC = C + 2;
    DFX_DYN_SMEM(float, sm);
    const int halo = DFX_CP_TT + A.kt - 1;
    const int CG = C / A.G, OG = A.NO / A.G;
    float *tile = sm;
    float *w1s = tile + halo * DFX_CP_FB * LDC;
    float *s1 = w1s + A.G * A.kt * CG * 16;
    const int tid = threadIdx.x, lane = tid & 63, wave = tid >> 6;
    int blk = blockIdx.x;
    const int fc = blk % A.fchunks;
    blk /= A.fchunks;
    const int tc = blk % A.tchunks;
    const int64_t b = blk / A.tchunks;
    const int64_t t0 = (int64_t)tc * DFX_CP_TT;
    const int f0 = fc * DFX_CP_FB;
    const int nt_valid = (int)((A.T - t0) < DFX_CP_TT ? (A.T - t0) : DFX_CP_TT);
    const int nf_valid = (A.Fd - f0) < DFX_CP_FB ? (A.Fd - f0) : DFX_CP_FB;
    for (int i = tid; i < A.G * A.kt * CG * 16; i += DFX_CP_THREADS) w1s[i] = A.w1[i];
    for (int i = tid; i < halo * DFX_CP_FB * C; i += DFX_CP_THREADS) {
        const int c = i % C;
        const int hf = i / C;
        const int f = hf % DFX_CP_FB, h = hf / DFX_CP_FB;
        const int64_t t = t0 - (A.kt - 1) + h;
        float v = 0.f;
        if (t >= 0 && t < A.T && f < nf_valid) v = A.c0[((b * A.T + t) * A.Fd + f0 + f) * C + c];
        tile[(h * DFX_CP_FB + f) * LDC + c] = v;
    }
    __syncthreads();
    const int nunits = DFX_CP_TT * A.G;
    for (int u = wave; u < nunits; u += DFX_CP_THREADS / 64) {
        const int tl = u / A.G, g = u - tl * A.G;
        f32x4 acc = f32x4{0.f, 0.f, 0.f, 0.f};
        for (int k = 0; k < A.kt; ++k) {
            const float *arow = tile + ((tl + k) * DFX_CP_FB + (lane & 15)) * LDC + g * CG + (lane >> 4);
            const float *brow = w1s + ((g * A.kt + k) * CG + (lane >> 4)) * 16 + (lane & 15);
            for (int ks = 0; ks < CG / 4; ++ks)
                acc = __builtin_amdgcn_mfma_f32_16x16x4f32(arow[4 * ks], brow[4 * ks * 16], acc, 0, 0, 0);
        }
        const int o = lane & 15;
        if (o < OG) {
#pragma unroll
            for (int r = 0; r < 4; ++r) {
                const int f = 4 * (lane >> 4) + r;
                s1[(tl * DFX_CP_FB + f) * A.NO + g * OG + o] = acc[r];
            }
        }
    }
    __syncthreads();
    for (int i = tid; i < DFX_CP_TT * DFX_CP_FB * A.NO; i += DFX_CP_THREADS) {
        const int n = i % A.NO;
// ... 2030 lines not shown
```

deepfilternet_amd/model.py:

```python
from __future__ import annotations

import ctypes as C
import glob
import os
import re
from typing import Dict, Optional, Tuple

import numpy as np
import torch

from . import _lib
from .config import ModelParams
from .libdf import DF

def make_cfg(p: ModelParams) -> _lib.ModelCfg:
    p.check_supported()
    return p.to_cfg()


def tensor_manifest(cfg: _lib.ModelCfg):
    L = _lib.lib()
    n = C.c_int()
    _lib.check(L.dfx_model_tensor_count(C.byref(cfg), C.byref(n)))
    out = []
# ... 9 lines not shown
def pack_state_dict(cfg: _lib.ModelCfg, sd: Dict[str, "np.ndarray | torch.Tensor"], strict: bool = True,
                    warn=None) -> np.ndarray:
    import warnings

    warn = warn or (lambda msg: warnings.warn(msg, stacklevel=3))
    total = C.c_int64()
    _lib.check(_lib.lib().dfx_model_blob_floats(C.byref(cfg), C.byref(total)))
    blob = np.zeros(total.value, dtype=np.float32)
    for name, shape, off in tensor_manifest(cfg):
        v = sd.get(name)
        if v is not None:
            v = v.detach().cpu().numpy() if isinstance(v, torch.Tensor) else np.asarray(v)
            if tuple(v.shape) != shape:
                if strict:
                    raise ValueError(f"size mismatch for {name}: checkpoint {tuple(v.shape)}, model {shape}")
                warn(f"size mismatch for {name}: copying a param with shape {tuple(v.shape)} from checkpoint, the shape in current "
                     f"model is {shape}. (dropped)")
                v = None
        elif strict:
            raise KeyError(f"state dict is missing '{name}'")
        else:
            warn(f"Missing key: '{name}'")
        n = int(np.prod(shape)) if shape else 1
        if v is None:
            leaf = name.rsplit(".", 1)[-1]
            is_bn = len(shape) == 1 and ".gru." not in name and "lsnr_fc" not in name
            fill = 1.0 if is_bn and leaf in ("weight", "running_var") else 0.0
            blob[off:off + n] = fill
        else:
            blob[off:off + n] = v.astype(np.float32, copy=False).ravel()
    return blob


class DfNet:

    def __init__(self, p: ModelParams, state_dict: Dict[str, "np.ndarray | torch.Tensor"], df_state: Optional[DF] = None,
                 run_df: bool = True, strict: bool = True):
        self.p = p
        self.cfg = make_cfg(p)
        blob = pack_state_dict(self.cfg, state_dict, strict=strict)
        h = C.c_void_p()
        _lib.check(_lib.lib().dfx_model_create(C.byref(self.cfg), blob.ctypes.data_as(C.POINTER(C.c_float)), C.byref(h)))
        self._h = h
        self.run_df = bool(run_df)
        if not self.run_df:
            _lib.check(_lib.lib().dfx_model_set_run_df(self._h, 0))
        self.df_state = df_state or DF(p.sr, p.fft_size, p.hop_size, p.nb_erb, p.min_nb_freqs)
        self.nb_df = p.nb_df
        self.df_order = p.df_order
        self.df_lookahead = p.df_lookahead
        self.freq_bins = p.freq_bins
        self.erb_bins = p.nb_erb
        self.post_filter = p.mask_pf
        self._ws: Optional[torch.Tensor] = None

    def __del__(self):
        h, self._h = getattr(self, "_h", None), None
        try:
            if h:
                _lib.lib().dfx_model_free(h)
        except Exception:
            pass

    @property
    def handle(self) -> C.c_void_p:
        return self._h

    def set_streams(self, enable: bool) -> None:
        _lib.check(_lib.lib().dfx_model_set_streams(self._h, int(bool(enable))))

    def set_pipeline(self, time_chunks: int = 6, min_chunk_frames: int = 32, batch_chunks: int = 1) -> None:
        _lib.check(_lib.lib().dfx_model_set_pipeline(self._h, int(time_chunks), int(min_chunk_frames), int(batch_chunks)))

    def check(self) -> None:
        _lib.check(_lib.lib().dfx_model_check(self._h))

    def poll(self) -> None:
        _lib.check(_lib.lib().dfx_model_poll(self._h))

    Q_GRU_PERSISTENT, Q_HWQ_PROBE, Q_EXACT_FP32, Q_SPIN_LIMIT, Q_PASSES_PERSISTENT, Q_PASSES_TICKET_BUSY = 1, 2, 3, 4, 5, 6
    Q_PASSES_C0_PRESPLIT = 7
    Q_LAST_PLAN = 8
    Q_PASSES_PAIR = 9
    PLAN_BITS = {"fan": 1 << 0, "fan_skp": 1 << 1, "fuse_h3": 1 << 2, "presplit": 1 << 3, "fuse_tail": 1 << 4, "fuse_enc": 1 << 5,
                 "fuse_enc4": 1 << 6, "enc_fan": 1 << 7, "dfenc": 1 << 8, "c0_fused": 1 << 9, "pipe": 1 << 10, "use_seq": 1 << 11,
                 "rows_finish": 1 << 14, "fuse_dec": 1 << 15}
    PLAN_DF_OUT_SHIFT, PLAN_DF_OUT_FORMS = 12, {0: "none", 1: "resident", 2: "streaming", 3: "ggemm"}

    def last_plan(self) -> Dict[str, object]:
        v = self.query(self.Q_LAST_PLAN)
        d: Dict[str, object] = {k: bool(v & b) for k, b in self.PLAN_BITS.items()}
        d["df_out"] = self.PLAN_DF_OUT_FORMS[(v >> self.PLAN_DF_OUT_SHIFT) & 3]
        return d

    def query(self, what: int) -> int:
        v = C.c_int64()
        _lib.check(_lib.lib().dfx_model_query(self._h, int(what), C.byref(v)))
        return int(v.value)

    def eval(self):
        return self

    def to(self, *a, **k):
        return self

    def workspace(self, nbytes: int) -> torch.Tensor:
        if self._ws is None or self._ws.numel() < nbytes or not _lib.on_device(self._ws):
            self._ws = None
            self._ws = torch.empty(int(nbytes), dtype=torch.uint8, device=_lib.device())
        return self._ws

    @torch.no_grad()
    def __call__(self, spec: torch.Tensor, feat_erb: torch.Tensor, feat_spec: torch.Tensor, atten_lim: float = 0.0
                 ) -> Tuple[torch.Tensor, torch.Tensor, torch.Tensor, torch.Tensor]:
        p = self.p
        dev = _lib.device()
        B, _, T, F, _ = spec.shape
        spec_d = spec.to(dev, torch.float32).contiguous()
        fe = feat_erb.to(dev, torch.float32).contiguous()
        fs = feat_spec.to(dev, torch.float32).contiguous()
        assert F == p.freq_bins and fe.shape == (B, 1, T, p.nb_erb) and fs.shape == (B, 1, T, p.nb_df, 2)
        spec_e = torch.empty_like(spec_d)
        m = torch.empty((B, 1, T, p.nb_erb), dtype=torch.float32, device=dev)
        lsnr = torch.empty((B, T, 1), dtype=torch.float32, device=dev)
        coefs = torch.empty((B, p.df_order, T, p.nb_df, 2), dtype=torch.float32, device=dev)
        nbytes = C.c_int64()
        L = _lib.lib()
        _lib.check(L.dfx_model_workspace_bytes(self._h, B, T, C.byref(nbytes)))
        ws = self.workspace(nbytes.value)
        _lib.check(L.dfx_model_forward(self._h, self.df_state.bands_handle, _lib.ptr(spec_d), _lib.ptr(fe), _lib.ptr(fs),
                                       B, T, float(atten_lim), _lib.ptr(spec_e), _lib.ptr(m), _lib.ptr(lsnr),
                                       _lib.ptr(coefs), _lib.ptr(ws), ws.numel(), _lib.stream()))
        if not self.run_df:
            coefs = torch.zeros((), device=dev)
        self.poll()
        return spec_e, m, lsnr, coefs

    forward = __call__


def _find_checkpoint(dirname: str, epoch) -> Tuple[Optional[str], int]:
    if not dirname or not os.path.isdir(dirname):
        return None, 0
    cps = glob.glob(os.path.join(dirname, "model_*.ckpt*"))
    if not cps:
        return None, 0

    def ep(path):
        mm = re.search(r"model_(\d+)\.ckpt", os.path.basename(path))
        return int(mm.group(1)) if mm else -1

    if isinstance(epoch, int) or (isinstance(epoch, str) and epoch.isdigit()):
        want = int(epoch)
        for c in cps:
            if ep(c) == want:
                return c, want
        return None, 0
    if epoch == "best":
        best = [c for c in cps if c.endswith(".best")]
        if best:
            c = max(best, key=ep)
            return c, ep(c)
    c = max(cps, key=ep)
    return c, ep(c)


# ... 75 lines not shown
```

include/dfx.h:

```cpp
#ifndef DFX_H
#define DFX_H

#include <stddef.h>
#include <stdint.h>

#ifdef __cplusplus
extern "C" {
#endif

#define DFX_OK 0
#define DFX_ERR_INVALID_ARG 1
#define DFX_ERR_UNSUPPORTED 2
#define DFX_ERR_HIP 3
#define DFX_ERR_NO_DEVICE 4
#define DFX_ERR_ALLOC 5

#define DFX_VERSION 200

#define DFX_G711_ULAW 1
#define DFX_G711_ALAW 2
#define DFX_FMT_F32 0
#define DFX_FMT_PCM16 1
#define DFX_FMT_ULAW 2
#define DFX_FMT_ALAW 3
// ... 11 lines not shown
int dfx_bands_nfreqs(const dfx_bands *b);

typedef struct dfx_state dfx_state;
int dfx_state_create(int sr, int fft_size, int hop_size, int nb_bands, int min_nb_erb_freqs, dfx_state **out);
void dfx_state_free(dfx_state *st);
int dfx_state_sr(const dfx_state *st);
int dfx_state_fft_size(const dfx_state *st);
int dfx_state_hop_size(const dfx_state *st);
int dfx_state_nb_erb(const dfx_state *st);
float dfx_state_wnorm(const dfx_state *st);
const dfx_bands *dfx_state_bands(const dfx_state *st);
int dfx_state_erb_widths(const dfx_state *st, uint64_t *out_host );
int dfx_state_fft_window(const dfx_state *st, float *out_host );
int dfx_erb_fb(int sr, int fft_size, int nb_bands, int min_nb_freqs, uint64_t *out_host);

int dfx_analysis(const dfx_state *st, const float *x, int64_t B, int64_t T, int64_t x_stride, const float *mem_in,
                 float *mem_out, float *spec, void *stream);

int dfx_synthesis(const dfx_state *st, const float *spec, int64_t B, int64_t Tf, const float *mem_in, float *mem_out,
                  float *out, int64_t out_stride, void *stream);

int dfx_erb(const dfx_bands *bands, const float *spec, int64_t rows, int db, float *out, void *stream);
int dfx_erb_inv(const dfx_bands *bands, const float *gains, int64_t rows, float *out, void *stream);
int dfx_erb_norm(float *x, int64_t C, int64_t T, int E, float alpha, float *state, void *stream);
int dfx_unit_norm(const float *x, int64_t x_frame_stride, float *out, int64_t C, int64_t T, int F, float alpha,
                  float *state, void *stream);
int dfx_unit_norm_init(int n, float *out_host);

int dfx_features(const dfx_state *st, const float *x, int64_t B, int64_t T, int64_t x_stride, int nb_df, float alpha,
                 float *spec, float *erb_feat, float *spec_feat, void *stream);

#define DFX_COEF_BOTF 0
#define DFX_COEF_BTFO 1
#define DFX_COEF_BTOF 2
int dfx_df_apply(const float *spec, const float *coefs, int coef_layout, const float *gains, const dfx_bands *bands,
                 int64_t B, int64_t T, int F, int nb_df, int order, int lookahead, float pf_beta, float atten_lim,
                 float *out, void *stream);
int dfx_df_apply_strided(const float *spec, int64_t spec_stride, const float *coefs, int coef_layout, const float *gains,
                         const dfx_bands *bands, int64_t B, int64_t T, int F, int nb_df, int order, int lookahead, float pf_beta,
                         float atten_lim, float *out, int64_t out_stride, void *stream);

#define DFX_SKIP_NONE 0
#define DFX_SKIP_IDENTITY 1
#define DFX_SKIP_GROUPEDLINEAR 2

typedef struct dfx_model_cfg {
    int32_t sr, fft_size, hop_size, nb_erb, nb_df, min_nb_freqs, df_order, df_lookahead;
    int32_t lsnr_min, lsnr_max;
    int32_t conv_lookahead, conv_ch, emb_hidden_dim, emb_num_layers, df_hidden_dim, df_num_layers;
    int32_t df_gru_skip;
    int32_t df_pathway_kernel_size_t, lin_groups, enc_lin_groups;
    int32_t mask_pf;
    float pf_beta;
    float norm_alpha;
    int32_t emb_gru_skip_enc, emb_gru_skip, enc_concat;
} dfx_model_cfg;

int dfx_model_tensor_count(const dfx_model_cfg *cfg, int *count);
int dfx_model_tensor_info(const dfx_model_cfg *cfg, int index, char *name_out, int name_cap, int64_t shape_out[4],
                          int *ndim_out, int64_t *offset_out );
int dfx_model_blob_floats(const dfx_model_cfg *cfg, int64_t *n);

typedef struct dfx_model dfx_model;
int dfx_model_create(const dfx_model_cfg *cfg, const float *blob_host, dfx_model **out);
void dfx_model_free(dfx_model *m);
int dfx_model_save_file(const dfx_model_cfg *cfg, const float *blob_host, const char *path);
int dfx_model_load_file(const char *path, dfx_model **out);
int dfx_onnx_targz_read(const char *path, dfx_model_cfg *cfg_out, float *blob_out, int64_t blob_cap, int64_t *blob_floats);
int dfx_model_cfg_get(const dfx_model *m, dfx_model_cfg *out);
int dfx_model_set_streams(dfx_model *m, int enable);
int dfx_model_set_run_df(dfx_model *m, int enable);
int dfx_model_set_pipeline(dfx_model *m, int time_chunks, int min_chunk_frames, int batch_chunks);
int dfx_model_poll(const dfx_model *m);
int dfx_model_check(const dfx_model *m);
#define DFX_Q_GRU_PERSISTENT 1
#define DFX_Q_HWQ_PROBE 2
#define DFX_Q_EXACT_FP32 3
#define DFX_Q_SPIN_LIMIT 4
#define DFX_Q_PASSES_PERSISTENT 5
#define DFX_Q_PASSES_TICKET_BUSY 6
#define DFX_Q_PASSES_C0_PRESPLIT 7
#define DFX_Q_PASSES_PAIR 9
#define DFX_Q_LAST_PLAN 8
#define DFX_PLAN_FAN (1 << 0)
#define DFX_PLAN_FAN_SKP (1 << 1)
#define DFX_PLAN_FUSE_H3 (1 << 2)
#define DFX_PLAN_PRESPLIT (1 << 3)
#define DFX_PLAN_FUSE_TAIL (1 << 4)
#define DFX_PLAN_FUSE_ENC (1 << 5)
#define DFX_PLAN_FUSE_ENC4 (1 << 6)
#define DFX_PLAN_ENC_FAN (1 << 7)
#define DFX_PLAN_DFENC (1 << 8)
#define DFX_PLAN_C0_FUSED (1 << 9)
#define DFX_PLAN_PIPE (1 << 10)
#define DFX_PLAN_USE_SEQ (1 << 11)
#define DFX_PLAN_DF_OUT_SHIFT 12
#define DFX_PLAN_DF_OUT_MASK (3 << DFX_PLAN_DF_OUT_SHIFT)
#define DFX_PLAN_DF_OUT_RESIDENT 1
#define DFX_PLAN_DF_OUT_STREAMING 2
#define DFX_PLAN_DF_OUT_GGEMM 3
#define DFX_PLAN_ROWS_FINISH (1 << 14)
#define DFX_PLAN_FUSE_DEC (1 << 15)
int dfx_model_query(const dfx_model *m, int what, int64_t *value);

int dfx_model_workspace_bytes(const dfx_model *m, int64_t B, int64_t T, int64_t *bytes);

int dfx_model_forward(const dfx_model *m, const dfx_bands *bands, const float *spec, const float *feat_erb,
                      const float *feat_spec, int64_t B, int64_t T, float atten_lim, float *spec_e, float *mask,
                      float *lsnr, float *df_coefs, void *workspace, int64_t workspace_bytes, void *stream);

int dfx_enhance_workspace_bytes(const dfx_model *m, const dfx_state *st, int64_t B, int64_t T, int pad, int64_t *bytes);
int dfx_enhance(const dfx_model *m, const dfx_state *st, const float *x, int64_t B, int64_t T, int pad,
                float atten_lim_db, float *y, void *workspace, int64_t workspace_bytes, void *stream);
int dfx_enhance_pcm16(const dfx_model *m, const dfx_state *st, const int16_t *x, int64_t B, int64_t T, int pad,
                      float atten_lim_db, int16_t *y, void *workspace, int64_t workspace_bytes, void *stream);
int dfx_enhance_varlen_workspace_bytes(const dfx_model *m, const dfx_state *st, int64_t B, const int64_t *lengths, int pad, int64_t *bytes);
int dfx_enhance_varlen(const dfx_model *m, const dfx_state *st, const float *x, int64_t B, int64_t x_stride, const int64_t *lengths,
                       int pad, float atten_lim_db, float *y, int64_t y_stride, void *workspace, int64_t workspace_bytes, void *stream);
int dfx_enhance_varlen_pcm16(const dfx_model *m, const dfx_state *st, const int16_t *x, int64_t B, int64_t x_stride, const int64_t *lengths,
                             int pad, float atten_lim_db, int16_t *y, int64_t y_stride, void *workspace, int64_t workspace_bytes, void *stream);

typedef struct dfx_stream_state dfx_stream_state;
int dfx_stream_create(const dfx_model *m, const dfx_state *st, int64_t streams, int max_frames, dfx_stream_state **out);
void dfx_stream_free(dfx_stream_state *s);
int dfx_stream_reset(dfx_stream_state *s, void *stream);
int dfx_stream_reset_streams(dfx_stream_state *s, const int64_t *ids, int64_t count, void *stream);
int dfx_stream_frames(const dfx_stream_state *s, int64_t *frames_out);
int dfx_stream_frame_length(const dfx_stream_state *s);
int dfx_stream_delay_frames(const dfx_stream_state *s);
int dfx_stream_set_atten_lim(dfx_stream_state *s, float lim_db);
int dfx_stream_set_atten_lim_enhance(dfx_stream_state *s, float atten_lim_db);
int dfx_stream_set_post_filter_beta(dfx_stream_state *s, float beta);
int dfx_stream_set_channels(dfx_stream_state *s, int channels, int reduce_mask);
int dfx_stream_set_gating(dfx_stream_state *s, int enable);
int dfx_stream_set_thresholds(dfx_stream_state *s, float min_db_thresh, float max_db_erb_thresh,
                              float max_db_df_thresh);
int dfx_stream_set_atten_lim_streams(dfx_stream_state *s, const int64_t *ids, int64_t count, const float *lim_db ,
                                     void *stream);
int dfx_stream_set_post_filter_beta_streams(dfx_stream_state *s, const int64_t *ids, int64_t count, const float *beta ,
                                            void *stream);
int dfx_stream_set_thresholds_streams(dfx_stream_state *s, const int64_t *ids, int64_t count, const float *thr ,
                                      void *stream);
int dfx_stream_get_settings(const dfx_stream_state *s, float *out_host);
int dfx_stream_process(dfx_stream_state *s, const float *x, int64_t n_frames, float *y, float *lsnr, void *stream);
int dfx_stream_set_pausable(dfx_stream_state *s, int enable);
int dfx_stream_process_active(dfx_stream_state *s, const float *x, int64_t n_frames, float *y, float *lsnr,
                              const unsigned char *active, void *stream);
int dfx_stream_process_raw(dfx_stream_state *s, const float *spec, float *gains, float *coefs, unsigned char *stages, float *lsnr,
                           void *stream);
int dfx_stream_set_sample_rate(dfx_stream_state *s, int sr, int lowpass_filter_width, double rolloff, int method, double beta);
int dfx_stream_sample_rate(const dfx_stream_state *s);
int64_t dfx_stream_resample_delay(const dfx_stream_state *s);
int dfx_stream_process_pcm16(dfx_stream_state *s, const int16_t *x, int64_t n_frames, int16_t *y, float *lsnr, const unsigned char *active,
                             void *stream);
int dfx_stream_process_g711(dfx_stream_state *s, const uint8_t *x, int law, int64_t n_frames, uint8_t *y, float *lsnr,
                            const unsigned char *active, void *stream);
int dfx_stream_process_ends(dfx_stream_state *s, const void *x, int x_format, int64_t n_frames, void *y, float *lsnr,
                            const int64_t *valid_hops, void *stream);
int dfx_stream_memory_bytes(const dfx_model *m, const dfx_state *st, int64_t streams, int max_frames, int64_t *bytes);
#define DFX_STREAM_META_MAGIC 0x53584644u
#define DFX_STREAM_META_VERSION 1u
typedef struct dfx_stream_meta {
    uint32_t magic, version;
    uint64_t fingerprint;
    int64_t age;
    float settings[5];
// ... 55 lines not shown
```

Measured before the change: 24.81 million frames/s.

## Precompute e0 skip contribution to mask in encoder instead of recomputing in tail

When e0 is not materialised (fused encoder and tail), the encoder kernels now compute the e0 skip path's contribution to the final mask conv (BN-scale, ReLU, 1x3 output projection via fp16-split MFMA) per frame and write a small per-row z0 vector. The ERB decoder tail then adds z0 to the mask logits instead of re-deriving e0 from the input features with a conv0 MFMA chain and then adding it channel-wise. Because the output conv is linear, the contribution can be moved. This removes redundant recomputation and per-channel work in the tail, at the cost of extra LDS tables and work in the encoder plus an R*E workspace buffer.

Result: no change. 24.74 million frames/s (-0.3%).

```diff
diff --git a/deepfilternet_amd/csrc/dfx_model.hip b/deepfilternet_amd/csrc/dfx_model.hip
--- a/deepfilternet_amd/csrc/dfx_model.hip
+++ b/deepfilternet_amd/csrc/dfx_model.hip
@@ -402,8 +402,8 @@
     PwW erb1, erb2, erb3, dfc0, dfc1, ct3, ct2, ct1;
     size_t co_w = 0, co_ska = 0, co_skb = 0;
     float co_bias = 0.f;
-    size_t tail_w0h3 = 0, tail_woh3 = 0;
-    float tail_w0_unscale = 1.f, tail_wo_unscale = 1.f;
+    size_t tail_woh3 = 0;
+    float tail_wo_unscale = 1.f;
     GlinW fc_emb, enc_in, enc_out, dec_in, dec_out, dfg_in, df_skip, df_out, enc_skip, dec_skip;
     std::vector<GruW> enc_gru, dec_gru, df_gru;
     size_t lsnr_w = 0;
@@ -442,6 +442,7 @@
     mutable int64_t passes_ps = 0;
     mutable int64_t passes_pair = 0;
     mutable int64_t last_plan = 0;
+    mutable int64_t last_z0 = -1;
     mutable int64_t passes_seq = 0, passes_ev = 0;
     mutable unsigned int seq_base = 0;
     unsigned long long *d_trace = nullptr;
@@ -894,11 +895,7 @@
     const int C = m->cfg.conv_ch;
     if (C % 32 != 0) return;
     const int KC = C / 32;
-    const size_t w0 = m->erb0_w, b0 = m->erb0_b, wo = m->co_w;
-    m->tail_w0h3 = pack_h3(P, C / 16, [&](int nt, int l, int i) {
-        const int k = 8 * (l >> 4) + i, ch = 16 * nt + (l & 15);
-        return k < 9 ? P.out[w0 + (size_t)k * C + ch] : (k == 9 ? P.out[b0 + ch] : 0.f);
-    }, &m->tail_w0_unscale);
+    const size_t wo = m->co_w;
     m->tail_woh3 = pack_h3(P, KC, [&](int kc, int l, int i) {
         const int j = l & 15, e = 8 * kc + i, ch = 16 * (e >> 2) + 4 * (l >> 4) + (e & 3);
         return j < 3 ? P.out[wo + (size_t)j * C + ch] : 0.f;
@@ -1230,6 +1227,7 @@
         case DFX_Q_SPIN_LIMIT: *value = m->spin_limit; return DFX_OK;
         case DFX_Q_PASSES_C0_PRESPLIT: *value = m->passes_ps; return DFX_OK;
         case DFX_Q_LAST_PLAN: *value = m->last_plan; return DFX_OK;
+        case DFX_Q_LAST_Z0: *value = m->last_z0; return DFX_OK;
         case DFX_Q_PASSES_PAIR: *value = m->passes_pair; return DFX_OK;
     }
     DFX_FAIL(DFX_ERR_INVALID_ARG, "dfx_model_query: unknown item %d", what);
@@ -1258,7 +1256,7 @@
 
 namespace {
 struct Ws {
-    size_t e0, e1, e2, e3, c0, c1, emb_in, emb, xa, xb, gi, xa2, xb2, gi2, demb, d3, d2, mask, c0p, xdf, coefs, lsnr, skp_e, skp_d, fps, total;
+    size_t e0, z0, e1, e2, e3, c0, c1, emb_in, emb, xa, xb, gi, xa2, xb2, gi2, demb, d3, d2, mask, c0p, xdf, coefs, lsnr, skp_e, skp_d, fps, total;
     size_t pgi[DFX_MAX_GRU_LAYERS], py[DFX_MAX_GRU_LAYERS], ph[DFX_MAX_GRU_LAYERS];
 };
 Ws plan_ws(const dfx_model *m, int64_t R, int64_t B) {
@@ -1273,6 +1271,7 @@
     };
     const size_t C = c.conv_ch, E = c.nb_erb, Fd = c.nb_df, emb = C * E / 4, NO = 2 * c.df_order;
     w.e0 = take(R * E * C);
+    w.z0 = take(R * E);
     w.e1 = take(R * (E / 2) * C);
     w.e2 = take(R * (E / 4) * C);
     w.e3 = take(R * (E / 4) * C);
diff --git a/deepfilternet_amd/csrc/dfx_model_forward.h b/deepfilternet_amd/csrc/dfx_model_forward.h
--- a/deepfilternet_amd/csrc/dfx_model_forward.h
+++ b/deepfilternet_amd/csrc/dfx_model_forward.h
@@ -41,7 +41,7 @@
     int Lk, E, Fd, O, NO, emb, L, kt;
     const int *tzr;
     Ws w{};
-    float *e0, *e1, *e2, *e3, *c0, *c1, *emb_in, *embv, *xa, *xb, *gi, *demb, *d3, *d2, *mask, *c0p, *xdf, *coefs, *lsnr, *xa2, *xb2, *gi2, *skp_e, *skp_d;
+    float *e0, *z0, *e1, *e2, *e3, *c0, *c1, *emb_in, *embv, *xa, *xb, *gi, *demb, *d3, *d2, *mask, *c0p, *xdf, *coefs, *lsnr, *xa2, *xb2, *gi2, *skp_e, *skp_d;
     bool run_df, fan, fan_skp, par, c0_fused, fuse_h3, fuse_tail, fuse_enc, no_e0, fuse_enc4, enc_fan, dfenc, pipe, use_seq;
     hipStream_t x1, x2;
     hipStream_t fin_s;
@@ -67,7 +67,7 @@
         sstride = fin ? fin->spec_stride : 0;
         fin_s = s;
         E = c.nb_erb, Fd = c.nb_df, O = c.df_order, NO = 2 * O, emb = C * E / 4, L = c.conv_lookahead;
-        e0 = ws + w.e0, e1 = ws + w.e1, e2 = ws + w.e2, e3 = ws + w.e3, c0 = ws + w.c0, c1 = ws + w.c1;
+        e0 = ws + w.e0, z0 = ws + w.z0, e1 = ws + w.e1, e2 = ws + w.e2, e3 = ws + w.e3, c0 = ws + w.c0, c1 = ws + w.c1;
         emb_in = ws + w.emb_in, embv = ws + w.emb, xa = ws + w.xa, xb = ws + w.xb, gi = ws + w.gi;
         demb = ws + w.demb, d3 = ws + w.d3, d2 = ws + w.d2;
         mask = mask_out ? mask_out : ws + w.mask;
@@ -90,6 +90,7 @@
         no_e0 = fuse_tail && fuse_enc;
         fuse_enc4 = m->can.erb_enc4 && !sc && !m->sw.erb_enc_split;
         e0r = no_e0 ? nullptr : e0;
+        m->last_z0 = no_e0 ? (int64_t)(w.z0 * sizeof(float)) : -1;
         if (sc && !fuse_enc) DFX_FAIL(DFX_ERR_UNSUPPORTED, "streaming needs the fused ERB encoder head (nb_erb even and <= 62, a frame's rows within the LDS)");
         gate = sc ? sc->gate : nullptr;
         if (gate && T - t_begin != 1) DFX_FAIL(DFX_ERR_INVALID_ARG, "gated streaming passes carry exactly one new frame");
@@ -201,7 +202,7 @@
     }
     int erb_dec_convs(int64_t M, DfxRowMap rm, hipStream_t st) {
         int r;
-        if (fuse_tail) return launch_erb_tail<C>(m, demb, e3, e2, e1, e0r, mask, M, E, st, rm, feat_erb, T, featT, Lk);
+        if (fuse_tail) return launch_erb_tail<C>(m, demb, e3, e2, e1, e0r, mask, M, E, st, rm, no_e0 ? z0 : nullptr);
         if ((r = launch_pw<C>(DFX_PW_MODE_DW3, m, m->ct3, demb, e3, d3, M, E / 4, E / 4, 1, st, rm))) return r;
         if ((r = launch_pw<C>(DFX_PW_MODE_DWT3, m, m->ct2, d3, e2, d2, M, E / 4, E / 2, 2, st, rm))) return r;
         return launch_erb_dec10<C>(m, d2, e1, e0, mask, M, E, st, rm);
@@ -308,9 +309,9 @@
     }
     int erb_range(int64_t t0, int64_t t1, int64_t Rk, DfxRowMap rm, hipStream_t st) {
         int r;
-        if (fuse_enc4) return launch_erb_enc4<C>(m, feat_erb, no_e0 ? nullptr : e0, e1, e2, e3, B, T, st, t0, Lk, t1, featT);
+        if (fuse_enc4) return launch_erb_enc4<C>(m, feat_erb, no_e0 ? nullptr : e0, e1, e2, e3, B, T, st, t0, Lk, t1, featT, no_e0 ? z0 : nullptr);
         if (fuse_enc) {
-            if ((r = launch_erb_enc<C>(m, feat_erb, no_e0 ? nullptr : e0, e1, B, T, st, t0, Lk, t1, featT))) return r;
+            if ((r = launch_erb_enc<C>(m, feat_erb, no_e0 ? nullptr : e0, e1, B, T, st, t0, Lk, t1, featT, no_e0 ? z0 : nullptr))) return r;
         } else {
             {
                 const int64_t total = R * E * (C / 4);
diff --git a/deepfilternet_amd/csrc/dfx_model_launch.h b/deepfilternet_amd/csrc/dfx_model_launch.h
--- a/deepfilternet_amd/csrc/dfx_model_launch.h
+++ b/deepfilternet_amd/csrc/dfx_model_launch.h
@@ -302,8 +302,7 @@
 
 template <int C>
 static int launch_erb_tail(const dfx_model *m, const float *demb, const float *e3, const float *e2, const float *e1, const float *e0,
-                           float *mask, int64_t R, int E, hipStream_t s, DfxRowMap rm, const float *feat_erb = nullptr, int64_t T = 0,
-                           int64_t feat_T = 0, int L = 0) {
+                           float *mask, int64_t R, int E, hipStream_t s, DfxRowMap rm, const float *z0 = nullptr) {
     if constexpr (C % 32 != 0) {
         DFX_FAIL(DFX_ERR_UNSUPPORTED, "erb tail: conv_ch");
     } else {
@@ -322,17 +321,14 @@
         A.skb[3] = m->p(m->co_skb);
         A.wo = m->p(m->co_w);
         A.woh3 = reinterpret_cast<const dfx_h8 *>(m->p(m->tail_woh3)), A.unscale_wo = m->tail_wo_unscale;
-        A.w0h3 = reinterpret_cast<const dfx_h8 *>(m->p(m->tail_w0h3)), A.unscale_w0 = m->tail_w0_unscale;
         A.bias_o = m->co_bias;
         A.out = mask;
         A.R = R;
         A.E = E;
         A.rm = rm;
         A.err = m->d_err;
-        if (!e0) {
-            if (!feat_erb || T <= 0) DFX_FAIL(DFX_ERR_INVALID_ARG, "erb tail: e0 or the features it is recomputed from");
-            A.feat = feat_erb, A.w0 = m->p(m->erb0_w), A.b0 = m->p(m->erb0_b), A.T = T, A.feat_T = feat_T, A.L = L;
-        }
+        A.z0 = z0;
+        if (!e0 && !z0) DFX_FAIL(DFX_ERR_INVALID_ARG, "erb tail: e0 or z0");
         const size_t smem = DFX_TAIL_SMEM(C);
         DFX_HIP(dfx_env_set_max_dyn_smem(e0 ? (const void *)dfx_k_erb_tail<C, false> : (const void *)dfx_k_erb_tail<C, true>, smem));
         DfxKScope ks(DFX_K_ERB_TAIL, s);
@@ -344,9 +340,19 @@
     }
 }
 
+template <int C, typename A_>
+static int erb_enc_z0_args(const dfx_model *m, float *z0, int E, A_ &A) {
+    if (!z0) return DFX_OK;
+    if (C % 32 != 0 || E != 32 || !m->can.pw_h3) DFX_FAIL(DFX_ERR_UNSUPPORTED, "erb encoder: z0 needs the fp16-split path, conv_ch %% 32 == 0, nb_erb 32");
+    A.z0 = z0;
+    A.ska0 = m->p(m->co_ska), A.skb0 = m->p(m->co_skb);
+    A.woh3 = reinterpret_cast<const dfx_h8 *>(m->p(m->tail_woh3)), A.unscale_wo = m->tail_wo_unscale;
+    return DFX_OK;
+}
+
 template <int C>
 static int launch_erb_enc(const dfx_model *m, const float *feat_erb, float *e0, float *e1, int64_t B, int64_t T, hipStream_t s,
-                          int64_t t_begin = 0, int L = -1, int64_t t_end = -1, int64_t feat_T = 0) {
+                          int64_t t_begin = 0, int L = -1, int64_t t_end = -1, int64_t feat_T = 0, float *z0 = nullptr) {
     const dfx_model_cfg &c = m->cfg;
     if (t_end < 0) t_end = T;
     DfxEncArgs A;
@@ -365,7 +371,8 @@
     A.E = c.nb_erb;
     A.L = L < 0 ? c.conv_lookahead : L;
     A.t_begin = t_begin;
-    const size_t smem = DFX_ENC_SMEM(C, c.nb_erb);
+    if (int r = erb_enc_z0_args<C>(m, z0, c.nb_erb, A)) return r;
+    const size_t smem = DFX_ENC_SMEM(C, c.nb_erb) + (z0 ? DFX_ENC_Z0_SMEM(C) : 0);
     DfxKScope ks(DFX_K_ERB_ENC, s);
     const dim3 grid((unsigned)nn_grid(dfx_ceil_div(B * (t_end - t_begin), 4), 2));
     if constexpr (C % 32 == 0) {
@@ -387,7 +394,7 @@
 
 template <int C>
 static int launch_erb_enc4(const dfx_model *m, const float *feat_erb, float *e0, float *e1, float *e2, float *e3, int64_t B, int64_t T,
-                           hipStream_t s, int64_t t_begin = 0, int L = -1, int64_t t_end = -1, int64_t feat_T = 0) {
+                           hipStream_t s, int64_t t_begin = 0, int L = -1, int64_t t_end = -1, int64_t feat_T = 0, float *z0 = nullptr) {
     if constexpr (C % 32 != 0) {
         DFX_FAIL(DFX_ERR_UNSUPPORTED, "erb enc4: conv_ch");
     } else {
@@ -415,6 +422,7 @@
         A.t_begin = t_begin;
         A.t_end = t_end;
         A.err = m->d_err;
+        if (int r = erb_enc_z0_args<C>(m, z0, c.nb_erb, A)) return r;
         const size_t smem = DFX_ENC4_SMEM(C, c.nb_erb);
         DFX_HIP(dfx_env_set_max_dyn_smem((const void *)dfx_k_erb_enc4<C>, smem));
         DfxKScope ks(DFX_K_ERB_ENC, s);
diff --git a/deepfilternet_amd/csrc/dfx_nn_kernels.h b/deepfilternet_amd/csrc/dfx_nn_kernels.h
--- a/deepfilternet_amd/csrc/dfx_nn_kernels.h
+++ b/deepfilternet_amd/csrc/dfx_nn_kernels.h
@@ -1624,6 +1624,68 @@
     if (H3 && amax >= DFX_H3_LIMIT && A.err) dfx_raise(A.err + 1);
 }
 
+#define DFX_Z0_TAB4(C) (2 * (C) / 4 + ((C) / 32) * 2 * 16)
+template <int C>
+static __device__ __forceinline__ void dfx_z0_tables(float4 *tab, const float *ska0, const float *skb0, const dfx_h8 *woh3, int tid, int nth) {
+    constexpr int C4 = C / 4, KC = C / 32;
+    dfx_h8 *wof = reinterpret_cast<dfx_h8 *>(tab + 2 * C4);
+    for (int i = tid; i < C4; i += nth) tab[i] = reinterpret_cast<const float4 *>(ska0)[i], tab[C4 + i] = reinterpret_cast<const float4 *>(skb0)[i];
+    for (int i = tid; i < KC * 2 * 16; i += nth) wof[i] = woh3[(i >> 4) * 64 + 16 * ((i & 15) >> 2) + (i & 3)];
+}
+template <int C>
+static __device__ __forceinline__ void dfx_z0_frame(float *e0s, const float4 *tab, float unscale_wo, float &amax, int lane, float *zout) {
+    constexpr int LD = C + 4, C4 = C / 4, NT = C / 16;
+    const dfx_h8 *wof = reinterpret_cast<const dfx_h8 *>(tab + 2 * C4);
+#pragma unroll
+    for (int t = 0; t < 2; ++t) {
+        int jl = lane & 15, q = lane >> 4;
+        DFX_OPAQUE(jl);
+        DFX_OPAQUE(q);
+        const int lw = 4 * q + (jl < 3 ? jl : 3);
+        float sv[8];
+        f32x4 va = f32x4{0.f, 0.f, 0.f, 0.f}, vb = va, vc = va;
+#pragma unroll
+        for (int nt = 0; nt < NT; ++nt) {
+            const float4 e = *reinterpret_cast<const float4 *>(e0s + (16 * t + jl) * LD + 16 * nt + 4 * q);
+            const float4 a = tab[4 * nt + q], b = tab[C4 + 4 * nt + q];
+            const int o = 4 * (nt & 1);
+            sv[o + 0] = fmaxf(a.x * e.x + b.x, 0.f), sv[o + 1] = fmaxf(a.y * e.y + b.y, 0.f);
+            sv[o + 2] = fmaxf(a.z * e.z + b.z, 0.f), sv[o + 3] = fmaxf(a.w * e.w + b.w, 0.f);
+            if (nt & 1) {
+                const int kc = nt >> 1;
+                dfx_h8 sh, sl;
+                dfx_split8_g(sv, sh, sl, amax);
+                const dfx_h8 woh = wof[(kc * 2 + 0) * 16 + lw], wol = wof[(kc * 2 + 1) * 16 + lw];
+                va = dfx_mfma_16x16x32_f16(wol, sh, va);
+                vb = dfx_mfma_16x16x32_f16(woh, sl, vb);
+                vc = dfx_mfma_16x16x32_f16(woh, sh, vc);
+            }
+        }
+        DFX_MFMA_GUARD();
+        const f32x4 vj = (va + vb) + vc;
+        if (lane < 16) {
+#pragma unroll
+            for (int j = 0; j < 3; ++j) {
+                const int i = jl * 3 + j;
+                e0s[(16 * t + (i >> 2)) * LD + C + (i & 3)] = vj[j] * unscale_wo;
+            }
+        }
+    }
+    DFX_WAVE_SYNC();
+    if (lane < 32) {
+        auto V = [&](int p, int j) -> float {
+            const int i = (p & 15) * 3 + j;
+            return e0s[(16 * (p >> 4) + (i >> 2)) * LD + C + (i & 3)];
+        };
+        int f = lane;
+        DFX_OPAQUE(f);
+        float z = V(f, 1);
+        if (f > 0) z += V(f - 1, 0);
+        if (f < 31) z += V(f + 1, 2);
+        zout[f] = z;
+    }
+}
+
 struct DfxEncArgs {
     const float *feat;
     const float *w0, *b0;
@@ -1636,10 +1698,15 @@
     float unscale = 1.f;
     unsigned int *err = nullptr;
     int64_t feat_T = 0;
+    float *z0 = nullptr;
+    const float *ska0 = nullptr, *skb0 = nullptr;
+    const dfx_h8 *woh3 = nullptr;
+    float unscale_wo = 1.f;
 };
 #define DFX_ENC_FS(E) (3 * ((E) + 2))
 #define DFX_ENC_WAVE_FLOATS(C, E) ((E) * ((C) + 4) + DFX_ENC_FS(E) + 2)
 #define DFX_ENC_SMEM(C, E) ((size_t)(3 * (C) / 4) * 16 + (size_t)4 * ((DFX_ENC_WAVE_FLOATS(C, E) + 3) / 4 * 4) * 4)
+#define DFX_ENC_Z0_SMEM(C) ((size_t)DFX_Z0_TAB4(C) * 16)
 
 template <int C, bool H3 = false>
 __global__ void __launch_bounds__(256, 2) dfx_k_erb_enc(DfxEncArgs A) {
@@ -1650,6 +1717,10 @@
     float4 *dws = sm4;
     float *s0 = reinterpret_cast<float *>(sm4 + 3 * C4) + (size_t)wave * ((DFX_ENC_WAVE_FLOATS(C, E) + 3) / 4 * 4);
     float *fs = s0 + E * LD;
+    constexpr bool can_z0 = H3 && C % 32 == 0;
+    float4 *z0t = sm4 + 3 * C4 + 4 * ((DFX_ENC_WAVE_FLOATS(C, E) + 3) / 4);
+    if constexpr (can_z0)
+        if (A.z0) dfx_z0_tables<C>(z0t, A.ska0, A.skb0, A.woh3, tid, 256);
     for (int i = tid; i < 3 * C4; i += 256) dws[i] = reinterpret_cast<const float4 *>(A.dw)[i];
     float a1[H3 ? 1 : NT][H3 ? 1 : CPL];
     dfx_h8 ahi[NT][KC], alo[NT][KC];
@@ -1704,6 +1775,9 @@
             *reinterpret_cast<float4 *>(s0 + p * LD + 4 * c4) = o;
         }
         DFX_WAVE_SYNC();
+        if constexpr (can_z0) {
+            if (A.z0) dfx_z0_frame<C>(s0, z0t, A.unscale_wo, amax, lane, A.z0 + r * 32);
+        }
         auto epi = [&](int p, bool valid, int nt, float4 o) {
             if (valid) *reinterpret_cast<float4 *>(A.e1 + (r * E1 + p) * C + 16 * nt + 4 * q) = o;
         };
@@ -1975,8 +2049,8 @@
 #define DFX_TAIL_WAVE_FLOATS(C) (32 * ((C) + 4))
 #define DFX_TAIL_TAB4(C) (3 * 3 * (C) / 4 + 4 * 2 * (C) / 4 + 3 * (C) / 4)
 #define DFX_TAIL_WFRAG(C) ((size_t)((C) / 16) * ((C) / 32) * 2 * 64)
-#define DFX_TAIL_W0_4(C) (((C) / 16) * 2 * 32 + ((C) / 32) * 2 * 16)
-#define DFX_TAIL_SMEM(C) ((size_t)(DFX_TAIL_TAB4(C) + DFX_TAIL_W0_4(C)) * 16 + 3 * DFX_TAIL_WFRAG(C) * 16 + (size_t)DFX_TAIL_WAVES * DFX_TAIL_WAVE_FLOATS(C) * 4)
+#define DFX_TAIL_WO4(C) (((C) / 32) * 2 * 16)
+#define DFX_TAIL_SMEM(C) ((size_t)(DFX_TAIL_TAB4(C) + DFX_TAIL_WO4(C)) * 16 + 3 * DFX_TAIL_WFRAG(C) * 16 + (size_t)DFX_TAIL_WAVES * DFX_TAIL_WAVE_FLOATS(C) * 4)
 static __host__ __device__ __forceinline__ bool dfx_tail_ok(int C, int E) {
     return (C == 32 || C == 64) && E == 32 && DFX_TAIL_SMEM(C) <= (size_t)160 * 1024;
 }
@@ -1988,18 +2062,14 @@
     const float *ska[4], *skb[4];
     const float *wo;
     const dfx_h8 *woh3;
-    const dfx_h8 *w0h3;
-    float unscale_wo, unscale_w0;
+    float unscale_wo;
     float bias_o;
     float *out;
     int64_t R;
     int E;
     DfxRowMap rm;
     unsigned int *err;
-    const float *feat = nullptr;
-    const float *w0 = nullptr, *b0 = nullptr;
-    int64_t T = 0, feat_T = 0;
-    int L = 0;
+    const float *z0 = nullptr;
 };
 template <int C, int MODE, int FB = C / 16, typename Epi>
 static __device__ __forceinline__ void dfx_chain_tile_h3_lds(const float *in, int Fin, int stride, int p0, int npos, const float4 *dws,
@@ -2069,7 +2139,7 @@
                         fmaxf(acc[nt][3] * unscale + bz.w, 0.f)));
     }
 }
-template <int C, bool RE0 = false>
+template <int C, bool Z0 = false>
 __global__ void __launch_bounds__(64 * DFX_TAIL_WAVES, 1) dfx_k_erb_tail(DfxTailArgs A) {
     constexpr int LD = C + 4, C4 = C / 4, NTH = 64 * DFX_TAIL_WAVES;
     constexpr int E = 32, E1 = 16, E4 = 8;
@@ -2077,13 +2147,12 @@
     constexpr int NV3 = (N3 + 63) / 64, NV1 = (N1 + 63) / 64, NV0 = (N0T + 63) / 64;
     DFX_DYN_SMEM(float4, sm4);
     const int tid = threadIdx.x, lane = tid & 63, wave = tid >> 6, q = lane >> 4;
-    constexpr int NT = C / 16, KC = C / 32;
+    constexpr int KC = C / 32;
     float4 *dws = sm4;
     float4 *sks = dws + 9 * C4;
     float4 *bis = sks + 8 * C4;
-    dfx_h8 *w0f = reinterpret_cast<dfx_h8 *>(bis + 3 * C4);
-    dfx_h8 *wof = w0f + NT * 2 * 32;
-    dfx_h8 *wfr = w0f + DFX_TAIL_W0_4(C);
+    dfx_h8 *wof = reinterpret_cast<dfx_h8 *>(bis + 3 * C4);
+    dfx_h8 *wfr = wof + DFX_TAIL_WO4(C);
     float *X = reinterpret_cast<float *>(wfr + 3 * DFX_TAIL_WFRAG(C)) + (size_t)wave * DFX_TAIL_WAVE_FLOATS(C);
     float *Y = X + 16 * LD;
 #pragma unroll
@@ -2092,16 +2161,13 @@
         for (int i = tid; i < C4; i += NTH) bis[l * C4 + i] = reinterpret_cast<const float4 *>(A.bias[l])[i];
         for (int i = tid; i < (int)DFX_TAIL_WFRAG(C); i += NTH) wfr[l * DFX_TAIL_WFRAG(C) + i] = A.wh3[l][i];
     }
-#pragma unroll
-    for (int pth = 0; pth < 4; ++pth)
+    constexpr bool z0f = Z0;
+#pragma unroll
+    for (int pth = 0; pth < (z0f ? 3 : 4); ++pth)
         for (int i = tid; i < C4; i += NTH) {
             sks[pth * 2 * C4 + i] = reinterpret_cast<const float4 *>(A.ska[pth])[i];
             sks[pth * 2 * C4 + C4 + i] = reinterpret_cast<const float4 *>(A.skb[pth])[i];
         }
-    constexpr bool re0 = RE0;
-    if (re0) {
-        for (int i = tid; i < NT * 2 * 32; i += NTH) w0f[i] = A.w0h3[(i >> 5) * 64 + (i & 31)];
-    }
     for (int i = tid; i < KC * 2 * 16; i += NTH) wof[i] = A.woh3[(i >> 4) * 64 + 16 * ((i & 15) >> 2) + (i & 3)];
     __syncthreads();
     const float4 *pd = reinterpret_cast<const float4 *>(A.demb), *p3 = reinterpret_cast<const float4 *>(A.e3), *p2 = reinterpret_cast<const float4 *>(A.e2),
@@ -2144,16 +2210,8 @@
             const int idx = l1 + 64 * i;
             r1[i] = idx < N1 ? p1[r * N1 + idx] : z4;
         }
-        float fxr[3] = {0.f, 0.f, 0.f};
-        if (re0) {
-            const uint32_t cb = (uint32_t)r / (uint32_t)A.T;
-            const int64_t ct = r - (int64_t)cb * A.T, fT = A.feat_T > 0 ? A.feat_T : A.T;
-#pragma unroll
-            for (int kt = 0; kt < 3; ++kt) {
-                const int64_t tau = ct - 2 + kt, tin = tau + A.L;
-                if (lane >= 1 && lane <= E && tau >= 0 && tin < A.T) fxr[kt] = A.feat[((int64_t)cb * fT + tin) * E + lane - 1];
-            }
-        }
+        float rz = 0.f;
+        if (z0f && l1 < E) rz = A.z0[r * E + l1];
         {
             const float4 a3 = sks[lq], b3 = sks[C4 + lq], a2 = sks[2 * C4 + lq], b2 = sks[3 * C4 + lq];
 #pragma unroll
@@ -2184,40 +2242,11 @@
         dfx_chain_tile_h3_lds<C, DFX_PW_MODE_DWT3>(X + E4 * LD, E4, 2, 0, E1, dws + 3 * C4, wfr + DFX_TAIL_WFRAG(C), bis + C4, A.unscale[1], amax, lane,
                                                    add_into(Y, 0));
         DFX_WAVE_SYNC();
-        const float4 a0 = sks[6 * C4 + lq], b0 = sks[7 * C4 + lq];
+        float4 a0 = z4, b0 = z4;
+        if constexpr (!z0f) a0 = sks[6 * C4 + lq], b0 = sks[7 * C4 + lq];
 #pragma unroll
         for (int t = 0; t < 2; ++t) {
-            if constexpr (re0) {
-                int jl = lane & 15;
-                DFX_OPAQUE(jl);
-                float xk[8];
-#pragma unroll
-                for (int i = 0; i < 8; ++i) xk[i] = __shfl(fxr[i / 3], 16 * t + jl + i % 3);
-                const float x8 = __shfl(fxr[2], 16 * t + jl + 2);
-#pragma unroll
-                for (int i = 0; i < 8; ++i) xk[i] = q == 0 ? xk[i] : 0.f;
-                if (q == 1) xk[0] = x8, xk[1] = 1.f;
-                dfx_h8 ph, pl;
-                dfx_split8_g(xk, ph, pl, amax);
-                int l32 = lane & 31;
-                DFX_OPAQUE(l32);
-                f32x4 acc0[NT];
-#pragma unroll
-                for (int nt = 0; nt < NT; ++nt) acc0[nt] = dfx_mfma_16x16x32_f16(w0f[(nt * 2 + 1) * 32 + l32], ph, f32x4{0.f, 0.f, 0.f, 0.f});
-#pragma unroll
-                for (int nt = 0; nt < NT; ++nt) acc0[nt] = dfx_mfma_16x16x32_f16(w0f[(nt * 2 + 0) * 32 + l32], pl, acc0[nt]);
-                DFX_OPAQUE(l32);
-#pragma unroll
-                for (int nt = 0; nt < NT; ++nt) acc0[nt] = dfx_mfma_16x16x32_f16(w0f[(nt * 2 + 0) * 32 + l32], ph, acc0[nt]);
-                DFX_MFMA_GUARD();
-#pragma unroll
-                for (int nt = 0; nt < NT; ++nt) {
-                    const float4 a0q = sks[6 * C4 + 4 * nt + q], b0q = sks[7 * C4 + 4 * nt + q];
-                    const float4 ev = make_float4(fmaxf(acc0[nt][0] * A.unscale_w0, 0.f), fmaxf(acc0[nt][1] * A.unscale_w0, 0.f),
-                                                  fmaxf(acc0[nt][2] * A.unscale_w0, 0.f), fmaxf(acc0[nt][3] * A.unscale_w0, 0.f));
-                    *reinterpret_cast<float4 *>(X + jl * LD + 16 * nt + 4 * q) = path(ev, a0q, b0q);
-                }
-            } else {
+            if constexpr (!z0f) {
 #pragma unroll
                 for (int i = 0; i < NV0; ++i) {
                     const int idx = lane + 64 * i;
@@ -2238,9 +2267,13 @@
             DFX_OPAQUE(lw);
             dfx_chain_tile_h3_lds<C, DFX_PW_MODE_DWT3, (C >= 64 ? C / 32 : C / 16)>(Y, E1, 2, 16 * t, E, dws + 6 * C4, wfr + 2 * DFX_TAIL_WFRAG(C), bis + 2 * C4, A.unscale[2], amax, lane,
                                                        [&](int p, bool, int nt, float4 d) {
-                                                           const float4 e = *reinterpret_cast<const float4 *>(X + (p - 16 * t) * LD + 16 * nt + 4 * q);
                                                            const int o = 4 * (nt & 1);
-                                                           sv[o + 0] = d.x + e.x, sv[o + 1] = d.y + e.y, sv[o + 2] = d.z + e.z, sv[o + 3] = d.w + e.w;
+                                                           if constexpr (z0f) {
+                                                               sv[o + 0] = d.x, sv[o + 1] = d.y, sv[o + 2] = d.z, sv[o + 3] = d.w;
+                                                           } else {
+                                                               const float4 e = *reinterpret_cast<const float4 *>(X + (p - 16 * t) * LD + 16 * nt + 4 * q);
+                                                               sv[o + 0] = d.x + e.x, sv[o + 1] = d.y + e.y, sv[o + 2] = d.z + e.z, sv[o + 3] = d.w + e.w;
+                                                           }
                                                            if (nt & 1) {
                                                                const int kc = nt >> 1;
                                                                dfx_h8 sh, sl;
@@ -2276,6 +2309,7 @@
             float acc = A.bias_o + V(f, 1);
             if (f > 0) acc += V(f - 1, 0);
             if (f < E - 1) acc += V(f + 1, 2);
+            if (z0f) acc += rz;
             A.out[r * E + f] = dfx_sigmoid(acc);
         }
         DFX_WAVE_SYNC();
@@ -2286,7 +2320,7 @@
 #define DFX_ENC4_WAVES 12
 #define DFX_ENC4_TAB4(C) (3 * 3 * (C) / 4 + 3 * (C) / 4)
 #define DFX_ENC4_WAVE_FLOATS(C, E) ((E) * ((C) + 4) + (DFX_ENC_FS(E) + 3) / 4 * 4)
-#define DFX_ENC4_SMEM(C, E) ((size_t)DFX_ENC4_TAB4(C) * 16 + 3 * DFX_TAIL_WFRAG(C) * 16 + (size_t)DFX_ENC4_WAVES * DFX_ENC4_WAVE_FLOATS(C, E) * 4)
+#define DFX_ENC4_SMEM(C, E) ((size_t)(DFX_ENC4_TAB4(C) + DFX_Z0_TAB4(C)) * 16 + 3 * DFX_TAIL_WFRAG(C) * 16 + (size_t)DFX_ENC4_WAVES * DFX_ENC4_WAVE_FLOATS(C, E) * 4)
 static __host__ __device__ __forceinline__ bool dfx_enc4_ok(int C, int E) {
     return (C == 32 || C == 64) && E == 32 && DFX_ENC4_SMEM(C, E) <= (size_t)160 * 1024;
 }
@@ -2302,6 +2336,10 @@
     int64_t t_begin, t_end;
     int64_t feat_T;
     unsigned int *err;
+    float *z0 = nullptr;
+    const float *ska0 = nullptr, *skb0 = nullptr;
+    const dfx_h8 *woh3 = nullptr;
+    float unscale_wo = 1.f;
 };
 template <int C, int N4>
 static __device__ __forceinline__ void dfx_enc4_store_rows(const float *strip, float4 *dst, int lane) {
@@ -2326,7 +2364,8 @@
     constexpr int E = 32, E1 = E / 2, E2 = E / 4, EP = E + 2;
     float4 *dws = sm4;
     float4 *bis = dws + 9 * C4;
-    dfx_h8 *wfr = reinterpret_cast<dfx_h8 *>(bis + 3 * C4);
+    float4 *z0t = bis + 3 * C4;
+    dfx_h8 *wfr = reinterpret_cast<dfx_h8 *>(z0t + DFX_Z0_TAB4(C));
     float *S0 = reinterpret_cast<float *>(wfr + 3 * DFX_TAIL_WFRAG(C)) + (size_t)wave * DFX_ENC4_WAVE_FLOATS(C, E);
     float *S1 = S0, *S2 = S0 + E1 * LD, *S3 = S2 + E2 * LD;
     float *fs = S0 + E * LD;
@@ -2336,6 +2375,7 @@
         for (int i = tid; i < C4; i += NTH) bis[l * C4 + i] = reinterpret_cast<const float4 *>(A.bias[l])[i];
         for (int i = tid; i < (int)DFX_TAIL_WFRAG(C); i += NTH) wfr[l * DFX_TAIL_WFRAG(C) + i] = A.wh3[l][i];
     }
+    if (A.z0) dfx_z0_tables<C>(z0t, A.ska0, A.skb0, A.woh3, tid, NTH);
     static_assert(64 % C4 == 0, "channel quad of a lane must not depend on the load index");
     constexpr int PP = E / (64 / C4);
     const int c4 = lane % C4, pbase = (lane / C4) * PP;
@@ -2405,6 +2445,7 @@
             }
         }
         DFX_WAVE_SYNC();
+        if (A.z0) dfx_z0_frame<C>(S0, z0t, A.unscale_wo, amax, lane, A.z0 + r * E);
         dfx_chain_tile_h3_lds<C, DFX_PW_MODE_DW3>(S0, E, 2, 0, E1, dws, wfr, bis, A.unscale[0], amax, lane, [=](int p, bool valid, int nt, float4 o) {
             if (nt == 0) DFX_WAVE_SYNC();
             if (valid) *reinterpret_cast<float4 *>(S1 + p * LD + 16 * nt + 4 * q) = o;
diff --git a/deepfilternet_amd/model.py b/deepfilternet_amd/model.py
--- a/deepfilternet_amd/model.py
+++ b/deepfilternet_amd/model.py
@@ -115,6 +115,7 @@
     Q_PASSES_C0_PRESPLIT = 7
     Q_LAST_PLAN = 8
     Q_PASSES_PAIR = 9
+    Q_LAST_Z0 = 10
     PLAN_BITS = {"fan": 1 << 0, "fan_skp": 1 << 1, "fuse_h3": 1 << 2, "presplit": 1 << 3, "fuse_tail": 1 << 4, "fuse_enc": 1 << 5,
                  "fuse_enc4": 1 << 6, "enc_fan": 1 << 7, "dfenc": 1 << 8, "c0_fused": 1 << 9, "pipe": 1 << 10, "use_seq": 1 << 11,
                  "rows_finish": 1 << 14, "fuse_dec": 1 << 15}
diff --git a/include/dfx.h b/include/dfx.h
--- a/include/dfx.h
+++ b/include/dfx.h
@@ -117,6 +117,7 @@
 #define DFX_Q_PASSES_C0_PRESPLIT 7
 #define DFX_Q_PASSES_PAIR 9
 #define DFX_Q_LAST_PLAN 8
+#define DFX_Q_LAST_Z0 10
 #define DFX_PLAN_FAN (1 << 0)
 #define DFX_PLAN_FAN_SKP (1 << 1)
 #define DFX_PLAN_FUSE_H3 (1 << 2)
```
